# schmeing/ReSeq

Hardware: AMD Instinct MI355X
Metric: simulated read-pairs/sec (2x150 bp) (higher is better)
Workload: dtype f64

## Files before the change

reseq_amd/csrc/rsq_core.h:

```cpp
#pragma once
#include "rsq_types.h"
#if !defined(__HIPCC_RTC__)
#include <math.h>
#endif

namespace rsq {

struct Words {
    uint32_t w0, w1, w2, w3;
};


RSQ_HD Words philox(uint64_t seed, uint32_t c0, uint32_t c1, uint32_t c2, uint32_t c3) {
    uint32_t k0 = (uint32_t)seed, k1 = (uint32_t)(seed >> 32);
#pragma unroll
    for (int r = 0; r < 10; ++r) {
        const uint64_t p0 = (uint64_t)0xD2511F53u * c0, p1 = (uint64_t)0xCD9E8D57u * c2;
        const uint32_t hi0 = (uint32_t)(p0 >> 32), lo0 = (uint32_t)p0, hi1 = (uint32_t)(p1 >> 32), lo1 = (uint32_t)p1;
        c0 = hi1 ^ c1 ^ k0;
        c1 = lo1;
        c2 = hi0 ^ c3 ^ k1;
        c3 = lo0;
        k0 += 0x9E3779B9u;
        k1 += 0xBB67AE85u;
// ... 359 lines not shown
RSQ_HD void surrounding_forward(const uint64_t *__restrict__ words, uint64_t word_off, uint32_t L, uint32_t pos, uint32_t (&sur)[3],
                                const uint64_t *__restrict__ wrap_words = nullptr) {
    uint64_t p = (uint64_t)pos + L - kSurStart;
    if (p >= L) p -= L;
    bool wrapped = pos < kSurStart;
    if (p + kSurBlocks * kSurRange <= L) {
        const uint64_t x = ref_bits60(words, word_off, (uint32_t)p);
#pragma unroll
        for (uint32_t b = 0; b < kSurBlocks; ++b) sur[b] = reverse_ten_bases((uint32_t)(x >> (20u * b)) & 0xFFFFFu);
        return;
    }
#pragma unroll 1
    for (uint32_t b = 0; b < kSurBlocks; ++b) {
        uint32_t v = 0;
#pragma unroll 1
        for (uint32_t i = 0; i < kSurRange; ++i) {
            v = (v << 2) + ref_base(wrapped && wrap_words ? wrap_words : words, word_off, (uint32_t)p);
            if (++p == L) {
                p = 0;
                wrapped = !wrapped;
            }
        }
        sur[b] = v;
    }
}
RSQ_HD void surrounding_reverse(const uint64_t *__restrict__ words, uint64_t word_off, uint32_t L, uint32_t pos, uint32_t (&sur)[3],
                                const uint64_t *__restrict__ wrap_words = nullptr) {
    uint64_t q = (uint64_t)(L - pos - 1) + L - kSurStart;
    if (q >= L) q -= L;
    uint32_t f = L - 1u - (uint32_t)q;
    bool wrapped = pos + kSurStart >= L;
    if (f + 1u >= kSurBlocks * kSurRange) {
        const uint64_t x = ref_bits60(words, word_off, f + 1u - kSurBlocks * kSurRange);
#pragma unroll
        for (uint32_t b = 0; b < kSurBlocks; ++b) sur[b] = ~(uint32_t)(x >> (20u * (kSurBlocks - 1u - b))) & 0xFFFFFu;
        return;
    }
#pragma unroll 1
    for (uint32_t b = 0; b < kSurBlocks; ++b) {
        uint32_t v = 0;
#pragma unroll 1
        for (uint32_t i = 0; i < kSurRange; ++i) {
            v = (v << 2) + (3u - ref_base(wrapped && wrap_words ? wrap_words : words, word_off, f));
            if (f) --f;
            else {
                f = L - 1u;
                wrapped = !wrapped;
            }
        }
        sur[b] = v;
    }
}
RSQ_HD double surrounding_bias(const double *__restrict__ sur_bias, const uint32_t (&sur)[3]) {
    double bias = 0.0;
    for (int b = (int)kSurBlocks; b--;) bias += sur_bias[(size_t)b * kSurSize + sur[b]];
    return 2 / (1 + exp(-bias));
}

RSQ_HD double get_dispersion(double bias, double a, double b) {
    double r = bias / (a + b * bias);
    if (r > bias * 1e10) r = bias * 1e10;
    return r;
}
RSQ_HD uint32_t binomial(uint32_t n, double p, double probability_chosen) {
    double probability_count = pow(1 - p, (double)n), probability_left = probability_chosen - probability_count;
    uint32_t count = 0;
    while (0.0 < probability_left && count < n) {
        ++count;
        probability_count *= (double)(n + 1 - count) / count * p / (1 - p);
        probability_left -= probability_count;
    }
    return count;
}
RSQ_HD uint32_t negative_binomial(double p, double r, double probability_chosen) {
    double probability_count = pow(1 - p, r), probability_left = probability_chosen - probability_count;
    uint32_t count = 0;
    while (0.0 < probability_left) {
        count = (count + 1u) & 0xFFFFu;
        probability_count *= p * ((r - 1) / count + 1);
        probability_left -= probability_count;
    }
    return count;
}
RSQ_HD uint32_t fragment_counts(const DevSim &S, uint32_t seq, uint32_t fragment_length, uint32_t gc, const uint32_t (&sur_start)[3],
                                const uint32_t (&sur_end)[3], double probability_chosen) {
    double general = S.ref_seq_bias[seq] * S.insert_lengths_bias[fragment_length];
    double bias = general * S.gc_bias[gc] * surrounding_bias(S.sur_bias, sur_start) * surrounding_bias(S.sur_bias, sur_end);
    if (0.0 < bias) {
        double mean = bias * S.bias_normalization;
        double dispersion = get_dispersion(mean, S.dispersion[0], S.dispersion[1]) / S.num_alleles;
        mean /= S.num_alleles;
        return negative_binomial(mean / (mean + dispersion), dispersion, probability_chosen);
    }
    return 0;
}


RSQ_HD uint32_t digits10(uint32_t v) { return v < 10 ? 1u : v < 100 ? 2u : v < 1000 ? 3u : v < 10000 ? 4u : 5u; }

struct CigarRun {
    char element;
    uint32_t length;
    uint32_t chars;
    RSQ_HD void flush() { chars += digits10(length) + 1u; }
};

struct FillState {
    uint32_t read_length, read_pos;
    uint32_t previous_indel_type, indel_pos, base_call, gc_seq;
    uint32_t seq_qual, qual, error_rate, num_errors;
    uint32_t last_written_qual;
    uint32_t iteration;
};

RSQ_HD uint32_t draw_read_length(const DevSim &S, uint32_t seg, uint32_t fragment_length, double u) {
    const DevReadLengths &rl = S.read_lengths[seg];
    if (rl.fixed) return rl.fixed;
    const double random_value = u * (double)S.insert_lengths[fragment_length];
    double counter = 0.0;
    const uint32_t row = fragment_length - rl.row_first;
    const uint32_t from = rl.row_from[row] & 0xFFFFu;
    uint32_t read_len = (from + (rl.row_ptr[row + 1] - rl.row_ptr[row])) & 0xFFFFu;
    while (counter <= random_value) {
        const bool more = read_len > from;
        read_len = (read_len - 1u) & 0xFFFFu;
        if (!more) break;
        counter += (double)rl.values[rl.row_ptr[row] + (read_len - from)];
    }
    return read_len;
}

template <class Src>
RSQ_HD void template_totals_loop(const Src &src, uint32_t n, uint32_t &gc, uint32_t &rate_sum) {
    for (uint32_t k = 0; k < n; ++k) {
        if (is_gc(src.base(k))) ++gc;
        rate_sum += src.sys_base(k) >> 8;
    }
}

struct AdapterSrc {
    const uint8_t *seq;
    const uint16_t *sys_;
    RSQ_HD uint32_t base(uint32_t k) const { return seq[k]; }
    RSQ_HD uint32_t sys_base(uint32_t k) const { return sys_[k]; }
    RSQ_HD uint32_t sys_deleted(uint32_t k) const { return sys_[k]; }
};

struct ReadMachine {
    enum : uint32_t { kTemplate = 0, kAdapter = 1, kTail = 2, kDone = 3 };
    FillState par;
    CigarRun cg;
    uint32_t phase, seg, tile_id, tbase;
    uint32_t org_pos, org_len;
    uint32_t adapter_id, adapter_a0;
    uint32_t iter_m, hard_clip, tail_length, pos_tail, n_indels;
    uint32_t start_cut_word;

    RSQ_HD void idle() {
        par = FillState{};
        cg = CigarRun{'M', 0, 0};
        phase = kDone;
        seg = tile_id = tbase = org_pos = org_len = adapter_id = adapter_a0 = iter_m = hard_clip = tail_length = pos_tail = n_indels = start_cut_word = 0;
    }
    template <class Tab, class Src>
    RSQ_HD void init(const DevSim &S, const Tab &tab, const Stream &st, uint32_t seg_, uint32_t tile, uint32_t fragment_length, const Src &src) {
        seg = seg_;
        tile_id = tile;
        tbase = (seg * RSQ_SIM(S, n_tiles) + tile_id) * 4u;
        par.read_pos = 0;
        par.previous_indel_type = 0;
        par.indel_pos = 0;
        par.base_call = 5;
        par.gc_seq = 0;
        par.qual = 1;
        par.error_rate = 0;
        par.num_errors = 0;
        par.last_written_qual = 0;
// ... 198 lines not shown
```

reseq_amd/csrc/rsq_format.h:

```cpp
#pragma once
#include <string.h>

#include "rsq_reads.h"

namespace rsq {

RSQ_HD void image_or(RSQ_LDS uint32_t *w, uint32_t v) {
#if defined(__HIP_DEVICE_COMPILE__)
    __hip_atomic_fetch_or(w, v, __ATOMIC_RELAXED, __HIP_MEMORY_SCOPE_WORKGROUP);
#else
    uint32_t x;
    memcpy(&x, w, 4);
    x |= v;
    memcpy(w, &x, 4);
#endif
}
RSQ_HD uint32_t image_bytes_at(uint32_t hi, uint32_t lo, uint32_t at) {
#if defined(__HIP_DEVICE_COMPILE__)
    return __builtin_amdgcn_perm(hi, lo, 0x03020100u + at * 0x01010101u);
#else
    return (uint32_t)((((uint64_t)hi << 32) | lo) >> (8u * at));
#endif
}
RSQ_HD uint32_t image_word(const uint32_t *p) {
// ... 343 lines not shown
    const uint64_t i = (uint64_t)blockIdx.x * blockDim.x + threadIdx.x;
    if (i >= n) return;
    const uint32_t seg = segs[i] ? 1u : 0u, fl = frag_len[i];
    if (fl < range.lo[seg] || fl >= range.hi[seg]) atomicMin(first_bad, (uint32_t)i);
}
__global__ void k_record_flags(const uint8_t *segs, uint64_t n, uint32_t *flags) {
    const uint64_t i = (uint64_t)blockIdx.x * blockDim.x + threadIdx.x;
    if (i < n) flags[i] = segs[i] ? 1u : 0u;
}
__global__ void k_record_partition(const uint8_t *segs, uint64_t n, const uint64_t *ones_before, uint32_t *rec_index, uint32_t *rec_count) {
    const uint64_t i = (uint64_t)blockIdx.x * blockDim.x + threadIdx.x;
    const uint32_t n1 = (uint32_t)ones_before[n], n0 = (uint32_t)n - n1;
    if (i == 0) {
        rec_count[0] = n0;
        rec_count[1] = n1;
    }
    if (i >= n) return;
    const uint32_t before = (uint32_t)ones_before[i];
    if (segs[i]) rec_index[n0 + before] = (uint32_t)i;
    else rec_index[(uint32_t)i - before] = (uint32_t)i;
}

__global__ void __launch_bounds__(256) k_methylation_templates(DevSim S, const Fragment *frags, uint64_t n_pairs, RawLayout raw) {
    const uint64_t r = (uint64_t)blockIdx.x * blockDim.x + threadIdx.x;
    if (r >= 2u * n_pairs) return;
    const uint32_t seg = r >= n_pairs ? 1u : 0u;
    convert_template(S, frags[r - seg * n_pairs], seg, raw.templates + r * raw.template_words, raw.template_words);
}

__global__ void __launch_bounds__(256) k_variant_templates(DevSim S, const Fragment *frags, const FragmentVar *fvars, uint64_t n_pairs, RawLayout raw) {
    const uint64_t r = (uint64_t)blockIdx.x * blockDim.x + threadIdx.x;
    if (r >= 2u * n_pairs) return;
    const uint32_t seg = r >= n_pairs ? 1u : 0u;
    const uint64_t pair = r - seg * n_pairs;
    variant_template(S, frags[pair], fvars[pair], seg, raw.templates + r * raw.template_words, raw.template_words);
}

template <bool PERM, uint32_t ITEMS>
struct WaveImage {
    const uint64_t *offsets;
    char *dst;
    uint32_t lane, skew, bytes, slot_at;
    uint64_t row, item, g_begin;
    bool active, through_lds;
    static __device__ __forceinline__ uint64_t first() { return (uint64_t)blockIdx.x * ITEMS; }
    __device__ __forceinline__ WaveImage(const uint64_t *offsets, uint64_t n, char *dst, uint32_t lds_bytes, const uint32_t *perm, uint32_t lane) : offsets(offsets), dst(dst), lane(lane) {
        const uint64_t last = first() + ITEMS < n ? first() + ITEMS : n;
        row = first() + (lane & (ITEMS - 1u));
        active = row < last;
        item = PERM ? (active ? perm[row] : 0u) : row;
        g_begin = PERM ? (active ? offsets[item] : 0u) : offsets[first()];
        const uint64_t g_end = PERM ? (active ? offsets[item + 1u] : 0u) : offsets[last];
        skew = (uint32_t)((uint64_t)(uintptr_t)(dst + g_begin) & 15u);
        bytes = (uint32_t)(g_end - g_begin);
        const uint32_t slot = (lds_bytes / ITEMS) & ~15u;
        through_lds = PERM ? __all(skew + bytes <= slot) != 0 : skew + bytes <= lds_bytes;
        slot_at = PERM ? (lane & (ITEMS - 1u)) * slot : 0u;
    }
    __device__ __forceinline__ RSQ_LDS char *item_text(char *image) const { return (RSQ_LDS char *)image + slot_at + skew + (PERM ? 0u : (uint32_t)(offsets[item] - g_begin)); }
    __device__ __forceinline__ void clear(char *image, uint32_t lds_bytes) const {
        for (uint32_t c = lane * 16u; c < lds_bytes; c += 64u * 16u) *reinterpret_cast<uint4 *>(image + c) = uint4{0u, 0u, 0u, 0u};
        __syncthreads();
    }
    __device__ __forceinline__ void store_out(const char *image) const {
        __syncthreads();
        const uint32_t lo = skew, hi = skew + bytes;
        char *g_chunk0 = dst + g_begin - skew;
        const char *s_from = image + slot_at;
        for (uint32_t c = (PERM ? lane / ITEMS : lane) * 16u; c < hi; c += (PERM ? 64u / ITEMS : 64u) * 16u) {
            if (c >= lo && c + 16u <= hi) {
                *reinterpret_cast<uint4 *>(g_chunk0 + c) = *reinterpret_cast<const uint4 *>(s_from + c);
            } else {
                for (uint32_t b = c < lo ? lo : c; b < c + 16u && b < hi; ++b) g_chunk0[b] = s_from[b];
            }
        }
    }
};

constexpr uint32_t kFormatLdsMax = 16u * 1024u, kFormatLdsMin = 1024u;
RSQ_HD uint32_t format_lds_bytes(uint64_t record_bytes, bool slots) {
    const uint64_t want = (kFormatRecords * record_bytes + 16u + 127u) & ~(uint64_t)127u;
    const uint32_t image = (uint32_t)(want < kFormatLdsMin ? kFormatLdsMin : want > kFormatLdsMax ? kFormatLdsMax : want);
    return !slots ? image : image + 16u * kFormatRecords < kFormatLdsMax ? image + 16u * kFormatRecords : kFormatLdsMax;
}
__global__ void __launch_bounds__(256) k_max_size(const uint32_t *sizes, uint64_t n, uint32_t *longest) {
    uint32_t m = 0;
    for (uint64_t i = (uint64_t)blockIdx.x * blockDim.x + threadIdx.x; i < n; i += (uint64_t)gridDim.x * blockDim.x) m = max(m, sizes[i]);
    for (uint32_t d = 32; d; d >>= 1) m = max(m, (uint32_t)__shfl_xor((int)m, (int)d, 64));
    if ((threadIdx.x & 63u) == 0 && m) atomicMax(longest, m);
}
template <bool PERM>
__global__ void __launch_bounds__(64) k_format_write(DevSim S, NameTable names, const Fragment *frags, uint64_t n_pairs, uint64_t adapter_only_first, RawLayout raw,
                                                    const uint64_t *offsets0, const uint64_t *offsets1, char *dst0, char *dst1, uint64_t cap0, uint64_t cap1,
                                                    const FragmentVar *fvars, const uint32_t *perm, uint32_t lds_bytes) {
    extern __shared__ __attribute__((aligned(16))) char s_text[];
    using Image = WaveImage<PERM, kFormatRecords>;
    const uint32_t lane = threadIdx.x, seg = blockIdx.y, part = lane / kFormatRecords;
    if (Image::first() >= n_pairs) return;
    const uint64_t *offsets = seg ? offsets1 : offsets0;
    char *dst = seg ? dst1 : dst0;
    if (offsets[n_pairs] > (seg ? cap1 : cap0)) return;
    const Image im(offsets, n_pairs, dst, lds_bytes, perm, lane);
    const uint64_t pair = im.item;
    ReadMeta m;
    Fragment f;
    FragmentVar fv;
    uint64_t r = 0;
    if (im.active) {
        r = (uint64_t)seg * n_pairs + im.row;
        m = raw.meta[r];
        if (frags) f = frags[pair];
        if (frags && fvars) fv = fvars[pair];
    }
    const WordColumn seq = raw.seq_of(r), qual = raw.qual_of(r), ops = raw.ops_of(r);
    const uint64_t ao_number = adapter_only_first + pair + 1u;
    if (!im.through_lds) {
        if (im.active && part == 0u) format_record(S, names, frags != nullptr, f, ao_number, m, seq, qual, ops, dst + offsets[pair], frags && fvars, fv);
        return;
    }
    im.clear(s_text, lds_bytes);
    if (im.active) {
        const uint32_t header = (uint32_t)(offsets[pair + 1u] - offsets[pair]) - 2u * m.read_len - 4u;
        image_record_part(m, seq, qual, header, part, im.item_text(s_text), [&](ImageSink &t) { image_header(S, names, frags != nullptr, f, ao_number, m, ops, t, frags && fvars, fv); });
    }
    im.store_out(s_text);
}

RSQ_HD uint32_t error_model_record_size(const ReadMeta &m, uint32_t id_len) { return 1u + id_len + 1u + m.cigar_chars + 2u + digits_u32(m.num_errors) + 1u + 2u * m.read_len + 4u; }
struct RecordIds {
    const char *chars;
    const uint64_t *off;
    const uint32_t *at, *len;
    RSQ_HD const char *begin(uint64_t i) const { return chars + (off ? off[i] : (uint64_t)at[i] + 1u); }
    RSQ_HD uint32_t length(uint64_t i) const { return off ? (uint32_t)(off[i + 1] - off[i]) : len[i]; }
};
__global__ void __launch_bounds__(256) k_record_text_sizes(RawLayout raw, uint64_t n, RecordIds ids, uint32_t *sizes) {
    const uint64_t row = (uint64_t)blockIdx.x * blockDim.x + threadIdx.x;
    if (row >= n) return;
    const uint64_t i = raw.item_of(row);
    sizes[i] = error_model_record_size(raw.meta[row], ids.length(i));
}
template <bool PERM>
__global__ void __launch_bounds__(64) k_record_text_waves(RawLayout raw, uint64_t n, RecordIds ids, const uint64_t *offsets, char *dst, uint64_t cap, uint32_t lds_bytes) {
    extern __shared__ __attribute__((aligned(16))) char s_text[];
    using Image = WaveImage<PERM, kFormatRecords>;
    const uint32_t lane = threadIdx.x, part = lane / kFormatRecords;
    if (Image::first() >= n || offsets[n] > cap) return;
    const Image im(offsets, n, dst, lds_bytes, raw.order, lane);
    const uint64_t row = im.row, item = im.item;
    const bool active = im.active;
    ReadMeta m{};
    if (active) m = raw.meta[row];
    const WordColumn seq = raw.seq_of(active ? row : 0u), qual = raw.qual_of(active ? row : 0u), ops = raw.ops_of(active ? row : 0u);
    auto header = [&](auto &t) {
        t.ch('@');
        t.str(ids.begin(item), ids.length(item));
        t.ch(' ');
        cigar_replay(ops, m, t);
        t.str(" E", 2);
        t.num((uint32_t)m.num_errors);
        t.ch('\n');
    };
    auto image_head = [&](ImageSink &t) {
        t.str(ids.begin(item), ids.length(item), '@', ' ');
        cigar_replay(ops, m, t);
        t.push(chars4(' ', 'E'), 2u);
        t.num((uint32_t)m.num_errors, '\n', 1u);
    };
    if (!im.through_lds) {
        if (active && part == 0u) {
            WordSinkT<char *> t(dst + offsets[item]);
            header(t);
// ... 18 lines not shown
```

reseq_amd/csrc/rsq_host.cpp:

```cpp
#include <stdio.h>
#include "rsq_host.h"
#include "rsq_textio.h"

#include <errno.h>
#include <fcntl.h>
#include <string.h>
#include <sys/mman.h>
#include <sys/stat.h>
#include <unistd.h>
#include <zlib.h>

#include <algorithm>
#include <array>
#include <atomic>
#include <chrono>
#include <exception>
#include <memory>
#include <mutex>

#include <fstream>
#include <thread>

#include "rsq_core.h"

namespace rsq {

Options &options() {
    static Options o;
    return o;
}
namespace {
struct OptionEntry {
    const char *name;
    int64_t Options::*field;
};
const OptionEntry kOptionTable[] = {
    {"fill_mode", &Options::fill_mode},         {"image_tiles", &Options::image_tiles},     {"rate_rows", &Options::rate_rows},
    {"no_indel_skip", &Options::no_indel_skip}, {"force_exact", &Options::force_exact},     {"min_quality_quads", &Options::min_quality_quads},
    {"trace_plan", &Options::trace_plan},       {"trace_prepare", &Options::trace_prepare},
    {"bias_window", &Options::bias_window},     {"window_chunks", &Options::window_chunks}, {"serial_fasta", &Options::serial_fasta},   {"trace_load", &Options::trace_load},
    {"chain_chunk", &Options::chain_chunk},     {"chain_warmup", &Options::chain_warmup},
    {"serial_parse", &Options::serial_parse},   {"parse_stretch", &Options::parse_stretch}, {"mapped_parses", &Options::mapped_parses},
    {"fasta_stretch", &Options::fasta_stretch}, {"overlap", &Options::overlap}, {"specialize", &Options::specialize}, {"job_write_direct", &Options::job_write_direct},             {"job_chunk_bytes", &Options::job_chunk_bytes}, {"host_gzip", &Options::host_gzip}, {"fill_waves", &Options::fill_waves}, {"fasta_no_stage", &Options::fasta_no_stage},
    {"hiprtc_by_name", &Options::hiprtc_by_name}, {"gzip_route", &Options::gzip_route},       {"gzip_stretch", &Options::gzip_stretch},
};
}
bool set_option(const char *name, int64_t value) {
    for (const OptionEntry &e : kOptionTable)
        if (0 == strcmp(name, e.name)) {
            options().*(e.field) = value;
            return true;
        }
    return false;
}
bool get_option(const char *name, int64_t *value) {
    for (const OptionEntry &e : kOptionTable)
        if (0 == strcmp(name, e.name)) {
            *value = options().*(e.field);
            return true;
        }
    return false;
}
const char *option_names() {
    static const std::string names = [] {
        std::string s;
        for (const OptionEntry &e : kOptionTable) s += (s.empty() ? "" : " ") + std::string(e.name);
        return s;
    }();
    return names.c_str();
}

static size_t pad8(size_t n) { return (8 - (n & 7)) & 7; }

Container::Container(const std::string &path) {
    std::ifstream f(path, std::ios::binary | std::ios::ate);
    if (!f) throw Error("cannot open profile '" + path + "'");
    std::streamsize sz = f.tellg();
    f.seekg(0);
    buf_.resize((size_t)sz);
    if (!f.read(reinterpret_cast<char *>(buf_.data()), sz)) throw Error("cannot read profile '" + path + "'");
    if (buf_.size() < 16 || memcmp(buf_.data(), "RSQPROF1", 8) != 0) throw Error("'" + path + "' is not an RSQP profile container");
    uint32_t version, n;
    memcpy(&version, &buf_[8], 4);
    memcpy(&n, &buf_[12], 4);
    if (version != 1) throw Error("unsupported RSQP version");
    static const size_t kSize[7] = {1, 2, 4, 8, 4, 8, 8};
    size_t pos = 16;
    for (uint32_t i = 0; i < n; ++i) {
        if (pos + 4 > buf_.size()) throw Error("truncated RSQP container");
        uint16_t ln;
        memcpy(&ln, &buf_[pos], 2);
        std::string name(reinterpret_cast<const char *>(&buf_[pos + 2]), ln);
        Array a;
        a.dtype = buf_[pos + 2 + ln];
        int ndim = buf_[pos + 3 + ln];
        if (a.dtype > 6 || ndim > 4) throw Error("corrupt RSQP container");
        size_t head = (size_t)ln + 4;
        pos += head + pad8(head);
        a.count = 1;
        for (int d = 0; d < ndim; ++d) {
            uint64_t dim;
            memcpy(&dim, &buf_[pos], 8);
            a.dims.push_back(dim);
            a.count *= dim;
            pos += 8;
        }
        size_t nbytes = a.count * kSize[a.dtype];
        if (pos + nbytes > buf_.size()) throw Error("truncated RSQP container");
        a.data = &buf_[pos];
        pos += nbytes + pad8(nbytes);
        arrays_[name] = a;
    }
}

const Array &Container::get(const std::string &name) const {
    auto it = arrays_.find(name);
    if (it == arrays_.end()) throw Error("profile misses array '" + name + "'");
    return it->second;
}

std::vector<double> discrete_cp(const uint64_t *w, size_t n) {
    std::vector<double> cp(n ? n : 1, 1.0);
    if (n < 2) return cp;
    double sum = 0.0;
    for (size_t i = 0; i < n; ++i) sum += (double)w[i];
    double acc = 0.0;
    for (size_t i = 0; i < n; ++i) {
// ... 1174 lines not shown
```

reseq_amd/csrc/rsq_host.h:

```cpp
#pragma once
#include <stdint.h>

#include <map>
#include <stdexcept>
#include <string>
#include <string.h>
#include <vector>

namespace rsq {

struct Error : std::runtime_error {
    using std::runtime_error::runtime_error;
};

struct Options {
    int64_t fill_mode = -1;
    int64_t image_tiles = 0;
    int64_t rate_rows = 0;
    int64_t no_indel_skip = 0;
    int64_t force_exact = 0;
    int64_t min_quality_quads = 0;
    int64_t trace_plan = 0;
    int64_t trace_prepare = 0;
    int64_t bias_window = 0;
    int64_t window_chunks = 0;
    int64_t trace_load = 0;
    int64_t serial_fasta = 0;
    int64_t fasta_stretch = 0;
    int64_t chain_chunk = 0;
    int64_t chain_warmup = -1;
    int64_t serial_parse = 0;
    int64_t mapped_parses = 0;
    int64_t parse_stretch = 0;
    int64_t job_chunk_bytes = 0;
    int64_t job_write_direct = 0;
    int64_t specialize = 1;
    int64_t fasta_no_stage = 0;
    int64_t fill_waves = 0;
    int64_t host_gzip = 0;
    int64_t gzip_route = -1;
    int64_t gzip_stretch = 0;
    int64_t hiprtc_by_name = 0;
    int64_t overlap = 0;
};
Options &options();
bool set_option(const char *name, int64_t value);
bool get_option(const char *name, int64_t *value);
const char *option_names();

struct Array {
    int dtype = 0;
    std::vector<uint64_t> dims;
    uint64_t count = 0;
    const uint8_t *data = nullptr;
};

class Container {
   public:
    explicit Container(const std::string &path);
    const Array &get(const std::string &name) const;
    bool has(const std::string &name) const { return arrays_.count(name) != 0; }
    template <class T>
    std::vector<T> vec(const std::string &name, int dtype) const {
        const Array &a = get(name);
        if (a.dtype != dtype) throw Error("profile array '" + name + "' has the wrong type");
        const T *p = reinterpret_cast<const T *>(a.data);
        return std::vector<T>(p, p + a.count);
    }
    template <class T>
    T scalar(const std::string &name, int dtype) const {
        return vec<T>(name, dtype).at(0);
    }

   private:
    std::vector<uint8_t> buf_;
    std::map<std::string, Array> arrays_;
};

template <class T>
struct Vect {
    uint64_t from = 0;
    std::vector<T> v;
    uint64_t to() const { return from + v.size(); }
    T operator[](uint64_t i) const { return (i < from || i >= to()) ? T(0) : v[i - from]; }
};

struct HostTable {
    uint32_t nm = 0;
    std::vector<uint32_t> par0;
    uint32_t from[4] = {0, 0, 0, 0}, to[4] = {0, 0, 0, 0};
    std::vector<double> dim2[4];
    void modify_par0(uint32_t par0_index, double multiplier);
    void set_par0(uint32_t par0_index);
};

struct HostAdapters {
    std::vector<uint8_t> seqs;
    std::vector<uint32_t> seq_ptr;
    std::vector<uint64_t> counts, significant;
    std::vector<uint32_t> cut_ptr, cut_from;
    std::vector<uint64_t> cut;
    uint32_t n() const { return (uint32_t)seq_ptr.size() - 1; }
};

struct HostRlByFl {
    uint64_t from = 0;
    std::vector<uint32_t> row_ptr, row_from;
    std::vector<uint64_t> values, non_mapped;
};

struct Profile {
    uint8_t phred_offset = 33;
    double corrected_coverage = 0;
    uint16_t max_len_deletion = 0;
    uint32_t reset_distance = 0;
    Vect<uint64_t> read_lengths[2];
    HostRlByFl rl_by_fl[2];
    uint64_t total_number_reads = 0;
    std::vector<uint16_t> tiles;
    std::vector<uint64_t> tile_abundance;
    HostAdapters adapters[2];
    Vect<uint64_t> polya;
    uint64_t overrun_bases[5] = {0, 0, 0, 0, 0};
    Vect<uint64_t> insert_lengths;
    Vect<double> insert_lengths_bias, gc_bias;
// ... 104 lines not shown
```

reseq_amd/csrc/rsq_scan.h:

```cpp
#pragma once
#include "rsq_types.h"

namespace rsq {

#if RSQ_DEVICE_BUILD
constexpr uint32_t kScanBlock = 256;
constexpr uint32_t kScanPer = 8;
constexpr uint32_t kScanTile = kScanBlock * kScanPer;

__global__ void k_scan_tile_sums(const uint32_t *in, uint64_t n, uint64_t *tile_sums) {
    __shared__ uint64_t s[kScanBlock];
    uint64_t base = (uint64_t)blockIdx.x * kScanTile + (uint64_t)threadIdx.x * kScanPer, acc = 0;
    for (uint32_t i = 0; i < kScanPer; ++i)
        if (base + i < n) acc += in[base + i];
    s[threadIdx.x] = acc;
    __syncthreads();
    for (uint32_t d = kScanBlock / 2; d > 0; d >>= 1) {
        if (threadIdx.x < d) s[threadIdx.x] += s[threadIdx.x + d];
        __syncthreads();
    }
    if (threadIdx.x == 0) tile_sums[blockIdx.x] = s[0];
}
constexpr uint32_t kScanTilesBlock = 1024;
__global__ void __launch_bounds__(kScanTilesBlock) k_scan_tiles(uint64_t *tile_sums, uint32_t n_tiles, uint64_t *total, const uint64_t *init) {
    __shared__ uint64_t s[kScanTilesBlock];
    const uint64_t first = init ? *init : 0u;
    const uint32_t per = (n_tiles + kScanTilesBlock - 1u) / kScanTilesBlock, lo = threadIdx.x * per, hi = lo + per < n_tiles ? lo + per : n_tiles;
    uint64_t acc = 0;
    for (uint32_t i = lo; i < hi; ++i) acc += tile_sums[i];
    s[threadIdx.x] = acc;
    __syncthreads();
    for (uint32_t d = 1; d < kScanTilesBlock; d <<= 1) {
        const uint64_t v = threadIdx.x >= d ? s[threadIdx.x - d] : 0;
        __syncthreads();
        s[threadIdx.x] += v;
        __syncthreads();
    }
    uint64_t run = first + s[threadIdx.x] - acc;
    for (uint32_t i = lo; i < hi; ++i) {
        const uint64_t v = tile_sums[i];
        tile_sums[i] = run;
        run += v;
    }
    if (threadIdx.x == kScanTilesBlock - 1u) *total = first + s[threadIdx.x];
}
__global__ void k_scan_apply(const uint32_t *in, uint64_t n, const uint64_t *tile_sums, const uint64_t *total, uint64_t *out) {
    __shared__ uint64_t s[kScanBlock];
    const uint64_t base = (uint64_t)blockIdx.x * kScanTile + (uint64_t)threadIdx.x * kScanPer;
    uint32_t v[kScanPer];
    uint64_t acc = 0;
    for (uint32_t i = 0; i < kScanPer; ++i) {
        v[i] = base + i < n ? in[base + i] : 0u;
        acc += v[i];
    }
    s[threadIdx.x] = acc;
    __syncthreads();
    for (uint32_t d = 1; d < kScanBlock; d <<= 1) {
        uint64_t t = threadIdx.x >= d ? s[threadIdx.x - d] : 0;
        __syncthreads();
        s[threadIdx.x] += t;
        __syncthreads();
    }
    uint64_t run = tile_sums[blockIdx.x] + s[threadIdx.x] - acc;
    for (uint32_t i = 0; i < kScanPer; ++i) {
        if (base + i < n) out[base + i] = run;
        run += v[i];
    }
    if (blockIdx.x == 0 && threadIdx.x == 0) out[n] = *total;
}
#endif

}
```

reseq_amd/csrc/rsq_sieve.h:

```cpp
#pragma once
#include "rsq_core.h"
#include "rsq_variants.h"

namespace rsq {

struct SieveSite {
    uint32_t seq, start, L;
    uint64_t word_off;
    const double *thr;
    uint32_t group;
    uint32_t sur_start[3];
    bool have_start;
    uint32_t sub;
    VarStart st;
};

RSQ_HD uint32_t site_c1(const SieveSite &site) { return site.seq | (site.sub << 22); }

template <class F>
RSQ_HD uint32_t sieve_gaps(const DevSim &S, const SieveSite &site, F &&on_pass) {
    const double *q = S.gap_q + (size_t)site.group * S.insert_to;
    const uint32_t *seg_end = S.gap_seg_end + (size_t)site.group * S.insert_to;
    const uint32_t c1 = site_c1(site);
    uint32_t cur = S.insert_from, k = 0, n = 0;
    while (cur < S.insert_to) {
        const Words w = philox(S.seed, site.start, c1, k++, kDomSieve << 28);
        const uint32_t e = seg_end[cur];
        const double base = (cur == S.insert_from || seg_end[cur - 1u] == cur) ? 1.0 : q[cur - 1u];
        const double target = u53_to_unit(w.w0, w.w1) * base;
        uint32_t lo = cur, hi = e;
        while (lo < hi) {
            const uint32_t mid = (lo + hi) >> 1;
            if (q[mid] <= target) hi = mid;
            else lo = mid + 1u;
        }
        if (lo < e) {
            const double thr1 = site.thr[2u * lo + 1u];
            on_pass(lo, thr1 + u53_to_unit(w.w2, w.w3) * (1 - thr1));
            ++n;
            cur = lo + 1u;
        } else cur = e;
    }
    return n;
}

RSQ_HD uint32_t sieve_cell(const DevSim &S, SieveSite &site, uint32_t len, double probability_chosen, uint32_t (&cnt)[2], uint32_t (&strand_of)[2]) {
    cnt[0] = cnt[1] = 0;
    strand_of[0] = strand_of[1] = 0;
    const double thr0 = site.thr[2u * len], thr1 = site.thr[2u * len + 1u];
    if (!(probability_chosen >= thr1)) return 0;
    const uint32_t non_zero_strands = binomial(2u, 1 - thr0, probability_chosen);
    const uint32_t end = site.start + len;
    if (!non_zero_strands || !(end < site.L)) return 0;
    const Words w2 = philox(S.seed, site.start, site.seq, len, (kDomSieve << 28) | 1u);
    uint32_t n_chosen;
    if (non_zero_strands <= 1u) {
        strand_of[0] = (uint32_t)(u32_to_unit(w2.w2) * 2.0) & 1u;
        n_chosen = 1;
    } else {
        strand_of[0] = 0;
        strand_of[1] = 1;
        n_chosen = 2;
    }
    if (!site.have_start) {
        surrounding_forward(S.ref_words, site.word_off, site.L, site.start, site.sur_start);
        site.have_start = true;
    }
    uint32_t sur_end[3];
    surrounding_reverse(S.ref_words, site.word_off, site.L, end - 1u, sur_end);
    const uint32_t gc = percent_u32(ref_gc_count_prefix(S.ref_words, S.gc_prefix, site.word_off, site.start, end), len);
    uint32_t n_here = 0;
    for (uint32_t j = 0; j < n_chosen; ++j) {
        const double u = j ? u53_to_unit(w2.w2, w2.w3) : u53_to_unit(w2.w0, w2.w1);
        const double adjusted_random = thr0 + u * (1 - thr0);
        cnt[j] = fragment_counts(S, site.seq, len, gc, site.sur_start, sur_end, adjusted_random);
        n_here += cnt[j];
    }
    return n_here;
}

constexpr uint32_t kMaxDevAlleles = 128;
template <uint32_t CAP>
struct VarCellT {
    uint32_t n;
    uint16_t cnt[2 * CAP];
    uint8_t id[2 * CAP];
};
using VarCell = VarCellT<kMaxDevAlleles>;
template <uint32_t CAP>
struct SlotMaskT {
    static constexpr uint32_t kWords = (2 * CAP + 31) / 32;
    uint32_t w[kWords];
    RSQ_HD void set_first(uint32_t n) {
        for (uint32_t i = 0; i < kWords; ++i) w[i] = n >= 32u * (i + 1u) ? 0xFFFFFFFFu : (n > 32u * i ? (1u << (n - 32u * i)) - 1u : 0u);
    }
    RSQ_HD bool test(uint32_t id) const { return (w[id >> 5] >> (id & 31u)) & 1u; }
    RSQ_HD void clear(uint32_t id) { w[id >> 5] &= ~(1u << (id & 31u)); }
};
template <class Mask>
RSQ_HD void select_allele(uint8_t *chosen, uint32_t &n_chosen, Mask &selectable, uint32_t possible_strands, double random_value) {
    uint32_t chosen_id = (uint32_t)(uint16_t)(random_value * (possible_strands - n_chosen));
    uint32_t replacement_correction = 0;
    for (uint32_t i = 0; i < n_chosen; ++i)
        if (chosen[i] <= chosen_id) ++replacement_correction;
    while (replacement_correction)
        if (selectable.test(++chosen_id)) --replacement_correction;
    chosen[n_chosen++] = (uint8_t)chosen_id;
    selectable.clear(chosen_id);
}
RSQ_HD uint32_t word_of(const Words &w, uint32_t k) { return k == 0u ? w.w0 : (k == 1u ? w.w1 : (k == 2u ? w.w2 : w.w3)); }
template <uint32_t CAP>
RSQ_HD uint32_t sieve_cell_var(const DevSim &S, const SieveSite &site, uint32_t len, double probability_chosen, VarCellT<CAP> &cell) {
    cell.n = 0;
    const double thr0 = site.thr[2u * len], thr1 = site.thr[2u * len + 1u];
    if (!(probability_chosen >= thr1)) return 0;
    const uint32_t possible_strands = 2u * S.num_alleles;
    const uint32_t non_zero_strands = binomial(possible_strands, 1 - thr0, probability_chosen);
    const uint32_t end = site.start + len;
    if (!non_zero_strands || !(end < site.L)) return 0;
    uint8_t chosen[2 * CAP];
    uint32_t n_chosen = 0, n_draws = 0;
    SlotMaskT<CAP> selectable;
    selectable.set_first(possible_strands);
    const bool direct = non_zero_strands <= possible_strands / 2u;
    const uint32_t to_draw = direct ? non_zero_strands : possible_strands - non_zero_strands;
    Words ws{0, 0, 0, 0};
    while (n_chosen < to_draw) {
        if (0u == (n_draws & 3u)) ws = philox(S.seed, site.start, site.seq, len, (kDomSieve << 28) | (2u + (n_draws >> 2)));
        select_allele(chosen, n_chosen, selectable, possible_strands, u32_to_unit(word_of(ws, n_draws & 3u)));
        ++n_draws;
    }
    if (!direct) {
        n_chosen = 0;
        for (uint32_t id = 0; id < possible_strands; ++id)
            if (selectable.test(id)) chosen[n_chosen++] = (uint8_t)id;
    }
    uint32_t n_here = 0;
    Words wc{0, 0, 0, 0};
#pragma unroll 1
    for (uint32_t j = 0; j < n_chosen; ++j) {
        const uint32_t allele = chosen[j] >> 1;
        const uint64_t *words = hap_words(S, allele);
        uint32_t sur_start[3], sur_end[3];
        surrounding_forward(words, site.word_off, site.L, site.start, sur_start, S.ref_words);
        surrounding_reverse(words, site.word_off, site.L, end - 1u, sur_end, S.ref_words);
        const uint32_t gc = percent_u32(ref_gc_count_prefix(words, hap_gc_prefix(S, allele), site.word_off, site.start, end), len);
        if (0u == (j & 1u)) wc = philox(S.seed, site.start, site.seq, len, (kDomSieve << 28) | (128u + (j >> 1)));
        const double u = (j & 1u) ? u53_to_unit(wc.w2, wc.w3) : u53_to_unit(wc.w0, wc.w1);
        const double adjusted_random = thr0 + u * (1 - thr0);
        const uint32_t c = fragment_counts(S, site.seq, len, gc, sur_start, sur_end, adjusted_random);
        if (c) {
            cell.id[cell.n] = chosen[j];
            cell.cnt[cell.n] = (uint16_t)c;
            ++cell.n;
            n_here += c;
        }
    }
    return n_here;
}

template <uint32_t CAP>
// ... 107 lines not shown
    if constexpr (VM != 2) {
        const uint32_t block_id = block_lo + slot / kBlockSize;
        init_site(S, block_id, slot % kBlockSize, site);
        if (first_slot_of_block) *first_slot_of_block = slot - slot % kBlockSize;
        return block_id;
    } else {
        const uint32_t base_lo = S.block_extra_ptr[block_lo];
        uint32_t lo = block_lo, hi = block_hi;
        while (hi - lo > 1u) {
            const uint32_t mid = (lo + hi) >> 1;
            if ((mid - block_lo) * kBlockSize + (S.block_extra_ptr[mid] - base_lo) <= slot) lo = mid;
            else hi = mid;
        }
        const uint32_t block_id = lo, first = (block_id - block_lo) * kBlockSize + (S.block_extra_ptr[block_id] - base_lo), local = slot - first;
        if (first_slot_of_block) *first_slot_of_block = first;
        const ExtraStart *e = S.extra + S.block_extra_ptr[block_id];
        const uint32_t m = S.block_extra_ptr[block_id + 1] - S.block_extra_ptr[block_id];
        const uint32_t seq = S.block_seq[block_id], bs = (block_id - S.first_block[seq]) * kBlockSize;
        uint32_t a = 0, b = m;
        while (a < b) {
            const uint32_t mid = (a + b) >> 1;
            if ((e[mid].pos - bs) + mid + 1u < local) a = mid + 1u;
            else b = mid;
        }
        const uint32_t c = a;
        if (c < m && (e[c].pos - bs) + c + 1u == local) {
            init_site(S, block_id, e[c].pos - bs, site);
            site.sub = e[c].sub;
            site.st = VarStart{e[c].first_variant_id, e[c].start_variant_pos};
        } else {
            init_site(S, block_id, local - c, site);
            if (NEED_START && site.start < site.L) site.st = VarStart{(int32_t)var_view(S, seq).lower_bound(site.start), 0u};
        }
        return block_id;
    }
}

#if RSQ_DEVICE_BUILD
constexpr uint32_t kSieveBlock = 256;

__global__ void __launch_bounds__(256) k_slot_table(DevSim S, uint32_t block_lo, SlotInfo *out) {
    const uint32_t block_id = block_lo + blockIdx.x, base_lo = S.block_extra_ptr[block_lo];
    const uint32_t first_slot = (block_id - block_lo) * kBlockSize + (S.block_extra_ptr[block_id] - base_lo);
    const ExtraStart *e = S.extra + S.block_extra_ptr[block_id];
    const uint32_t m = S.block_extra_ptr[block_id + 1] - S.block_extra_ptr[block_id];
    const uint32_t seq = S.block_seq[block_id], bs = (block_id - S.first_block[seq]) * kBlockSize, L = S.seq_len[seq];
    const VarView r = var_view(S, seq);
    __shared__ uint32_t s_v[2];
    if (threadIdx.x < 2) s_v[threadIdx.x] = r.lower_bound(bs + threadIdx.x * kBlockSize);
    __syncthreads();
    const uint32_t v0 = s_v[0], v1 = s_v[1];
    for (uint32_t local = threadIdx.x; local < kBlockSize + m; local += blockDim.x) {
        uint32_t a = 0, b = m;
        while (a < b) {
            const uint32_t mid = (a + b) >> 1;
            if ((e[mid].pos - bs) + mid + 1u < local) a = mid + 1u;
            else b = mid;
        }
        SlotInfo t;
        t.block_id = block_id;
        t.first_slot = first_slot;
        if (a < m && (e[a].pos - bs) + a + 1u == local) {
            t.offset_in_block = e[a].pos - bs;
            t.sub = e[a].sub;
            t.first_variant_id = e[a].first_variant_id;
            t.start_variant_pos = e[a].start_variant_pos;
        } else {
            t.offset_in_block = local - a;
            t.sub = 0;
            const uint32_t pos = bs + t.offset_in_block;
            uint32_t lo = v0, hi = v1;
            while (lo < hi) {
                const uint32_t mid = (lo + hi) >> 1;
                if (r.v[mid].pos < pos) lo = mid + 1u;
                else hi = mid;
            }
            t.first_variant_id = pos < L ? (int32_t)lo : 0;
            t.start_variant_pos = 0;
        }
        out[first_slot + local] = t;
    }
}

template <int VM, bool FILL>
__global__ void __launch_bounds__(kSieveBlock) k_sieve_gaps(DevSim S, uint32_t block_lo, uint32_t block_hi, uint32_t n_slots, uint32_t *counts, const uint64_t *cand_off,
                                                            SieveCand *cands, uint64_t cand_cap, const SlotInfo *slots) {
    const uint32_t slot = blockIdx.x * kSieveBlock + threadIdx.x;
    if (slot >= n_slots) return;
    SieveSite site;
    init_site_slot<VM, false>(S, block_lo, block_hi, slot, site, nullptr, slots);
    if (!(site.start < site.L)) {
        if constexpr (!FILL) counts[slot] = 0;
        return;
    }
    if constexpr (FILL) {
        uint64_t at = cand_off[slot];
        sieve_gaps(S, site, [&](uint32_t len, double probability_chosen) {
            if (at < cand_cap) cands[at] = SieveCand{slot, len, probability_chosen};
            ++at;
        });
    } else counts[slot] = sieve_gaps(S, site, [](uint32_t, double) {});
}

template <int VM, uint32_t CAP = kMaxDevAlleles>
__global__ void __launch_bounds__(kSieveBlock) k_sieve_finish(DevSim S, uint32_t block_lo, uint32_t block_hi, uint32_t n_slots, const uint64_t *cand_off, const SieveCand *cands,
                                                              uint64_t cand_cap, uint32_t *pairs_of, SieveHit *hits, uint32_t hit_cap, uint32_t *hit_count, const SlotInfo *slots,
                                                              uint32_t *cell_info) {
    __shared__ uint32_t s_records, s_base;
    if (threadIdx.x == 0) s_records = 0;
    __syncthreads();
    const uint64_t c = (uint64_t)blockIdx.x * kSieveBlock + threadIdx.x;
    const bool has_cell = c < cand_cap && c < cand_off[n_slots];
    uint32_t n_here = 0, n_records = 0;
    SieveCand cand{};
    VarCellT<VM != 0 ? CAP : 1u> cell;
    cell.n = 0;
    if (has_cell) {
        cand = cands[c];
        SieveSite site;
        init_site_slot<VM>(S, block_lo, block_hi, cand.slot, site, nullptr, slots);
        if constexpr (VM == 2) n_here = sieve_cell_general(S, site, cand.len, cand.probability_chosen, cell);
        else if constexpr (VM == 1) n_here = sieve_cell_var(S, site, cand.len, cand.probability_chosen, cell);
        else {
            uint32_t cnt[2], strand_of[2];
            n_here = sieve_cell(S, site, cand.len, cand.probability_chosen, cnt, strand_of);
            cell.n = n_here ? 2u : 0u;
            for (uint32_t e = 0; e < 2u; ++e) {
                cell.cnt[e] = (uint16_t)cnt[e];
                cell.id[e] = (uint8_t)strand_of[e];
            }
        }
        n_records = (cell.n + 1u) / 2u;
    }
    if constexpr (VM == 0) {
        if (c < cand_cap) {
            pairs_of[c] = n_here;
            cell_info[c] = (uint32_t)cell.cnt[0] | ((uint32_t)(cell.id[0] & 1u) << 16) | ((uint32_t)(cell.id[1] & 1u) << 17);
        }
        return;
    }
    const uint32_t rank = n_records ? atomicAdd(&s_records, n_records) : 0u;
    __syncthreads();
    if (threadIdx.x == 0 && s_records) s_base = atomicAdd(hit_count, s_records);
    __syncthreads();
    uint32_t intra = 0;
    for (uint32_t e = 0; e < cell.n; e += 2u) {
        const bool two = e + 1u < cell.n;
        const uint32_t at = s_base + rank + e / 2u;
        SieveHit h;
        h.slot = cand.slot;
        h.cand = (uint32_t)c;
        h.intra = intra;
        h.len = (uint16_t)cand.len;
        h.cnt0 = cell.cnt[e];
        h.cnt1 = two ? cell.cnt[e + 1u] : (uint16_t)0;
        h.strand0 = cell.id[e] & 1u;
        h.allele0 = cell.id[e] >> 1;
        h.strand1 = two ? cell.id[e + 1u] & 1u : 0;
        h.allele1 = two ? cell.id[e + 1u] >> 1 : 0;
        if (at < hit_cap) hits[at] = h;
        intra += (uint32_t)h.cnt0 + h.cnt1;
    }
    if (c < cand_cap) pairs_of[c] = n_here;
}

template <int VM>
__global__ void __launch_bounds__(256) k_sieve_emit(DevSim S, uint32_t block_lo, uint32_t block_hi, const SieveHit *hits, uint32_t n_hits, const uint64_t *cand_off,
                                                   const uint64_t *pair_off, Fragment *frags, FragmentVar *fvars, const SlotInfo *slots, const SieveCand *cands = nullptr,
                                                   const uint32_t *pairs_of = nullptr, const uint32_t *cell_info = nullptr) {
    const uint32_t i = blockIdx.x * blockDim.x + threadIdx.x;
    if (i >= n_hits) return;
    SieveHit h;
    if constexpr (VM == 0) {
        const uint32_t pairs = pairs_of[i];
        if (!pairs) return;
        const SieveCand cand = cands[i];
        const uint32_t info = cell_info[i];
        h.slot = cand.slot;
        h.cand = i;
        h.intra = 0;
        h.len = (uint16_t)cand.len;
        h.cnt0 = (uint16_t)(info & 0xFFFFu);
        h.cnt1 = (uint16_t)(pairs - (info & 0xFFFFu));
        h.strand0 = (uint8_t)((info >> 16) & 1u);
        h.strand1 = (uint8_t)((info >> 17) & 1u);
        h.allele0 = h.allele1 = 0;
    } else h = hits[i];
    SieveSite site;
    uint32_t first_slot;
    const uint32_t block_id = init_site_slot<VM>(S, block_lo, block_hi, h.slot, site, &first_slot, slots);
    const uint64_t base = pair_off[h.cand];
    const uint32_t number_base = (uint32_t)(base - pair_off[cand_off[first_slot]]);
    uint32_t k = h.intra;
    for (uint32_t e = 0; e < 2u; ++e) {
        const uint32_t cnt = e ? h.cnt1 : h.cnt0, strand = e ? h.strand1 : h.strand0, allele = e ? h.allele1 : h.allele0;
        if (!cnt) continue;
        FragmentVar fv{};
        if constexpr (VM == 2) {
            const AlleleCell ac = allele_cell(allele_view(S, site.seq, allele), site.st, site.start, h.len);
            fv.end = ac.end;
            fv.sub = site.sub;
            fv.start_var = site.st.first_variant_id;
            fv.start_var_pos = site.st.start_variant_pos;
            fv.end_var = ac.end_var.first_variant_id;
            fv.end_var_pos = ac.end_var.start_variant_pos;
        }
        for (uint32_t dup = 0; dup < cnt; ++dup, ++k) {
            frags[base + k] = make_fragment(site, h.len, dup, strand, block_id, number_base + k + 1u, allele);
// ... 8 lines not shown
```

reseq_amd/csrc/rsq_sim.hip:

```cpp
#include <hip/hip_runtime.h>
#include <fcntl.h>
#include <sys/mman.h>
#include <sys/stat.h>
#include <math.h>
#include <string.h>
#include <unistd.h>

#include <algorithm>
#include <atomic>
#include <chrono>
#include <map>
#include <thread>
#include <memory>
#include <string>
#include <utility>
#include <vector>

#include "../../include/reseq_amd.h"
#include "rsq_deflate.h"
#include "rsq_fasta.h"
#include "rsq_chains.h"
#include "rsq_sieve.h"
#include "rsq_scan.h"
#include "rsq_text.h"
#include "rsq_reads.h"
#include "rsq_format.h"
#include "rsq_sam.h"
#include "rsq_bam.h"
#include "rsq_bamsort.h"
#include "rsq_pack.h"
#include "rsq_prepass.h"
#include "rsq_spec.h"
#include "rsq_textio.h"

namespace rsq {

static thread_local std::string g_last_error, g_last_warning;

struct HipError : Error {
    using Error::Error;
};
#define HIP_CHECK(expr)                                                                                       \
    do {                                                                                                      \
        hipError_t e_ = (expr);                                                                               \
        if (e_ != hipSuccess) throw HipError(std::string(#expr) + ": " + hipGetErrorString(e_));              \
    } while (0)

class DevBuf {
   public:
    DevBuf() = default;
    DevBuf(const DevBuf &) = delete;
    DevBuf &operator=(const DevBuf &) = delete;
    DevBuf(DevBuf &&o) noexcept : p_(o.p_), bytes_(o.bytes_) { o.p_ = nullptr; o.bytes_ = 0; }
    ~DevBuf() { if (p_) (void)hipFree(p_); }
    void reserve(size_t bytes) {
        if (bytes <= bytes_) return;
        if (p_) {
            HIP_CHECK(hipDeviceSynchronize());
            HIP_CHECK(hipFree(p_));
        }
        p_ = nullptr;
        bytes_ = 0;
        HIP_CHECK(hipMalloc(&p_, bytes ? bytes : 8));
        bytes_ = bytes;
    }
    template <class T>
    void upload(const std::vector<T> &v) {
        reserve(v.size() * sizeof(T) + 8);
        if (!v.empty()) HIP_CHECK(hipMemcpy(p_, v.data(), v.size() * sizeof(T), hipMemcpyHostToDevice));
    }
    void release() {
        if (p_) {
            HIP_CHECK(hipDeviceSynchronize());
            HIP_CHECK(hipFree(p_));
        }
        p_ = nullptr;
        bytes_ = 0;
    }
    void reserve_keeping(size_t bytes, size_t keep, hipStream_t st) {
        if (bytes <= bytes_) return;
        DevBuf bigger;
        bigger.reserve(bytes);
        if (keep) HIP_CHECK(hipMemcpyAsync(bigger.p_, p_, keep, hipMemcpyDeviceToDevice, st));
        HIP_CHECK(hipStreamSynchronize(st));
        std::swap(p_, bigger.p_);
        std::swap(bytes_, bigger.bytes_);
    }
    template <class T>
    T *as() const { return reinterpret_cast<T *>(p_); }
    size_t bytes() const { return bytes_; }

   private:
    void *p_ = nullptr;
    size_t bytes_ = 0;
};

}
#include "rsq_s2i.h"
namespace rsq {

struct Timer {
    std::vector<std::pair<hipEvent_t, hipEvent_t>> events;
    size_t used = 0;
    Timer() = default;
    Timer(const Timer &) = delete;
    Timer &operator=(const Timer &) = delete;
    ~Timer() {
        for (auto &e : events) {
            (void)hipEventDestroy(e.first);
            (void)hipEventDestroy(e.second);
        }
    }
    void reset() { used = 0; }
    void start(hipStream_t st) {
        if (used == events.size()) {
            hipEvent_t a, b;
            HIP_CHECK(hipEventCreate(&a));
            HIP_CHECK(hipEventCreate(&b));
            events.emplace_back(a, b);
        }
        HIP_CHECK(hipEventRecord(events[used].first, st));
    }
    void stop(hipStream_t st) {
        HIP_CHECK(hipEventRecord(events[used].second, st));
        ++used;
    }
    double ms() const {
        double sum = 0.0;
        for (size_t i = 0; i < used; ++i) {
            float t = 0;
            if (hipEventElapsedTime(&t, events[i].first, events[i].second) == hipSuccess) sum += t;
        }
        return sum;
    }
    size_t launches() const { return used; }
};

}

using namespace rsq;

struct rsq_profile {
    Profile p;
};
struct rsq_ref {
    Reference r;
    Variants variants;
    bool has_variants = false;
};

struct DeviceUploader : Uploader {
    std::vector<std::unique_ptr<DevBuf>> owned[kUploadScopes];
    int device = 0;
    void bind_thread() override { HIP_CHECK(hipSetDevice(device)); }
    void release_scope(int scope) override {
        HIP_CHECK(hipDeviceSynchronize());
        owned[scope].clear();
    }
    void *put_bytes(const void *data, size_t bytes) override {
        std::vector<std::unique_ptr<DevBuf>> &own = owned[current_scope];
        own.emplace_back(new DevBuf());
        own.back()->reserve(bytes + 8);
        HIP_CHECK(hipMemcpy(own.back()->as<void>(), data, bytes, hipMemcpyHostToDevice));
        return own.back()->as<void>();
    }
    void *put_zeros(size_t bytes) override {
        std::vector<std::unique_ptr<DevBuf>> &own = owned[current_scope];
        own.emplace_back(new DevBuf());
        own.back()->reserve(bytes + 8);
        HIP_CHECK(hipMemset(own.back()->as<void>(), 0, bytes + 8));
        return own.back()->as<void>();
    }
    void write_bytes(void *dst, const void *src, size_t bytes) override { HIP_CHECK(hipMemcpy(dst, src, bytes, hipMemcpyHostToDevice)); }
    void read_bytes(void *dst_host, const void *src, size_t bytes) override { HIP_CHECK(hipMemcpy(dst_host, src, bytes, hipMemcpyDeviceToHost)); }
};

struct MappedFile {
    const char *data = nullptr;
    size_t size = 0;
    explicit MappedFile(const char *path) {
        const int fd = open(path, O_RDONLY);
        if (fd < 0) throw Error(std::string("cannot open ") + path + ": " + strerror(errno));
        struct stat st;
        if (fstat(fd, &st) != 0 || st.st_size <= 0) {
            close(fd);
            throw Error(std::string(path) + " is empty or cannot be examined");
        }
        size = (size_t)st.st_size;
        void *p = mmap(nullptr, size, PROT_READ, MAP_PRIVATE, fd, 0);
        close(fd);
        if (p == MAP_FAILED) throw Error(std::string("cannot map ") + path);
        data = static_cast<const char *>(p);
    }
    ~MappedFile() {
        if (data) munmap(const_cast<char *>(data), size);
    }
    MappedFile(const MappedFile &) = delete;
    MappedFile &operator=(const MappedFile &) = delete;
};

struct rsq_sim : PrepassSim {
    int device = 0;
    DeviceUploader up;
    struct Workspace {
        DevBuf fvars;
        DevBuf slot_table;
        DevBuf counts, offsets, tile_sums, scan_total, frags, raw_seq, raw_qual, raw_ops, raw_meta, sizes, off_r1, off_r2, fill_counters, hits, hit_count, cands, pairs_of, pair_off, templates, rec_flags, rec_index, rec_count;
        DevBuf bin_keys, bin_small, bin_perm, bin_frags, bin_fvars;
        DevBuf fa_counts, fa_first, fa_at, fa_len, fa_id_len, fa_frag_len, fa_seg, fa_codes, fa_summary;
        DevBuf sam_sizes, sam_side, off_sam;
        DevBuf bam_side;
        DevBuf cell_info;
        hipEvent_t text_done = nullptr;
    } ws[2];
    struct JobText {
        std::vector<std::unique_ptr<DevBuf>> chunks[2];
        std::vector<size_t> used[2];
        uint64_t bytes[2] = {0, 0};
        bool complete = false;
        std::vector<unsigned char> packed[2];
        bool is_packed = false;
        bool device_packed = false;
        void clear() {
            complete = false;
            is_packed = false;
            device_packed = false;
            for (auto &p : packed) std::vector<unsigned char>().swap(p);
            for (int f = 0; f < 2; ++f) {
                chunks[f].clear();
                used[f].clear();
                bytes[f] = 0;
            }
        }
    } job;
    DevBuf totals;
    bool gz_dense = false;
    bool gz_keep_code = false, gz_have_code = false;
    DevBuf gz_slots, gz_sizes, gz_at, gz_hist, gz_codes, gz_total;
    Workspace *cur = &ws[0];
    hipStream_t side[2] = {nullptr, nullptr};
    hipEvent_t ev_call = nullptr, ev_fill = nullptr, ev_emit = nullptr;
    std::map<std::string, Timer> timers;
    uint32_t n_cu = 256;
    uint64_t *mailbox = nullptr;
    uint64_t format_record_bytes = 480;
    DevBuf longest_record;
    DevBuf sam_totals, sam_longest;
    uint64_t sam_pair_bytes = 1100;
    uint64_t bam_pair_bytes = 700;
    struct BamSorted {
        bool active = false;
        uint64_t stream_at = 0;
        uint32_t next_block = 0;
        uint64_t prev_cut = 0;
        BamSortPlan plan{};
        DevBuf stage[2], dir[2];
        int cur = 0;
        uint64_t n_held = 0, held_bytes = 0;
        uint64_t call_pairs = 0;
        uint32_t call_parts = 1;
        DevBuf keys[2], idx[2], hist, hist_at, sizes, at, flags, run_of, runs, result, out_of_order, windows, window_first;
        BamIndexState index;
    } bam_sorted;
    uint64_t record_text_bytes = 480;
    int force_fill_mode = -1;
    SpecKernels spec;
    std::string arch;
    bool specialize = true;
    struct ChainBufs {
        DevBuf chains, chunk_chain, used, out[2], changed, list;
    } chain_bufs;
};

static bool fill_is_binned(const rsq_sim &s) { return effective_fill_mask(s.dev.lds.mask, s.force_fill_mode) != 0 && s.dev.lds.binned; }
static thread_local std::string g_spec_note;
static hipFunction_t spec_kernel(rsq_sim &s, SpecKind kind, uint32_t mask, bool var, bool binned) {
    if (!s.specialize || mask == 0) return nullptr;
    std::string note;
    hipFunction_t fn = s.spec.get(s.dev, SpecVariant{kind, mask, var, binned}, s.arch, note);
    if (s.opt.trace_plan && note != g_spec_note) fprintf(stderr, "[rsq] %s\n", note.c_str());
    g_spec_note = note;
    return fn;
}

namespace rsq {

constexpr uint64_t kBiasWindow = 512ull << 20;
struct DevicePrepass : PrepassBackend {
    rsq_sim &s;
    hipStream_t st;
    DevicePrepass(rsq_sim &sim, void *stream) : s(sim), st((hipStream_t)stream) {}

    void bias_partials(const BiasPlan &plan, uint64_t g_lo, uint64_t g_hi, std::vector<double> &h_sum, std::vector<double> &h_max) override {
        const bool trace = s.opt.trace_prepare != 0;
        auto t0 = std::chrono::steady_clock::now();
        auto lap = [&](const char *what) {
            if (!trace) return;
            HIP_CHECK(hipStreamSynchronize(st));
            const auto t1 = std::chrono::steady_clock::now();
            fprintf(stderr, "prepare:   bias sums: %-18s %8.3f s\n", what, std::chrono::duration<double>(t1 - t0).count());
            t0 = t1;
        };
        const uint32_t n_chunks = bias_chunks(plan);
        if (!n_chunks) return;
        DevBuf d_params, d_chunk_param, d_chunk_ptr, d_sum, d_max, d_start_bias, d_end_bias;
        d_params.upload(plan.params);
        d_chunk_param.upload(plan.chunk_param);
        d_chunk_ptr.upload(plan.chunk_ptr);
        d_sum.reserve((size_t)n_chunks * 8);
        d_max.reserve((size_t)n_chunks * 8);
        HIP_CHECK(hipMemsetAsync(d_sum.as<double>(), 0, (size_t)n_chunks * 8, st));
        HIP_CHECK(hipMemsetAsync(d_max.as<double>(), 0, (size_t)n_chunks * 8, st));
        lap("chunk tables");
        const uint64_t lo = std::min<uint64_t>(g_lo, s.total_ref_size), hi = std::min<uint64_t>(g_hi, s.total_ref_size);
        uint64_t window = kBiasWindow;
        if (s.opt.bias_window > 0) window = (uint64_t)s.opt.bias_window;
        const uint64_t reach = (uint64_t)kBiasBlock * kBiasRun + s.dev.insert_to, track_len = std::min(hi - lo, window) + reach;
        d_start_bias.reserve(track_len * 8 + 16);
        d_end_bias.reserve(track_len * 8 + 16);
        lap("track buffers");
        for (uint64_t a = lo; a < hi; a += window) {
            const uint64_t b = std::min(hi, a + window), w_hi = std::min<uint64_t>(s.total_ref_size, b + reach);
            hipLaunchKernelGGL(k_surrounding_bias_tracks, dim3((uint32_t)cdiv(w_hi - a, 256)), dim3(256), 0, st, s.dev, d_start_bias.as<double>(), d_end_bias.as<double>(), a, w_hi);
            HIP_CHECK(hipGetLastError());
            hipLaunchKernelGGL(k_sum_bias, dim3(n_chunks), dim3(kBiasBlock), 0, st, s.dev, d_params.as<BiasParam>(), d_chunk_param.as<uint32_t>(), d_chunk_ptr.as<uint32_t>(),
                               d_start_bias.as<double>(), d_end_bias.as<double>(), a, d_sum.as<double>(), d_max.as<double>(), a, b);
            HIP_CHECK(hipGetLastError());
        }
        lap("track and sum kernels");
        HIP_CHECK(hipMemcpyAsync(h_sum.data(), d_sum.as<double>(), h_sum.size() * 8, hipMemcpyDeviceToHost, st));
        HIP_CHECK(hipMemcpyAsync(h_max.data(), d_max.as<double>(), h_max.size() * 8, hipMemcpyDeviceToHost, st));
        HIP_CHECK(hipStreamSynchronize(st));
        lap("download");
    }

    void begin_run(const ChainRun &run, const std::vector<uint32_t> &chunk_chain) override {
        rsq_sim::ChainBufs &b = s.chain_bufs;
        publish_chains(run);
        b.chunk_chain.upload(chunk_chain);
        b.used.reserve(run.n_chunks * 4);
        b.out[0].reserve(run.n_chunks * 4);
        b.out[1].reserve(run.n_chunks * 4);
        b.changed.reserve(8);
        b.list.reserve((size_t)run.n_chunks * 4 + 16);
    }
    void publish_chains(const ChainRun &run) override { s.chain_bufs.chains.upload(run.chains); }
    uint32_t run_pass(const ChainRun &run, uint32_t pass, int prev, int cur) override {
        rsq_sim::ChainBufs &b = s.chain_bufs;
        uint32_t *out_prev = b.out[prev].as<uint32_t>(), *out_new = b.out[cur].as<uint32_t>();
        uint32_t n_run = run.n_chunks;
        const uint32_t *list = nullptr;
        if (pass > 0) {
            HIP_CHECK(hipMemsetAsync(b.changed.as<uint32_t>(), 0, 4, st));
            hipLaunchKernelGGL(k_sys_chain_select, dim3(cdiv(run.n_chunks, 256)), dim3(256), 0, st, b.chains.as<Chain>(), b.chunk_chain.as<uint32_t>(), run.n_chunks,
                               b.used.as<uint32_t>(), out_prev, out_new, b.list.as<uint32_t>(), b.changed.as<uint32_t>(), (int)pass);
            HIP_CHECK(hipGetLastError());
            HIP_CHECK(hipMemcpyAsync(&n_run, b.changed.as<uint32_t>(), 4, hipMemcpyDeviceToHost, st));
            HIP_CHECK(hipStreamSynchronize(st));
            list = b.list.as<uint32_t>();
        }
        if (n_run) {
            hipLaunchKernelGGL(k_sys_chain, dim3(cdiv(n_run, 64)), dim3(64), 0, st, s.dev, b.chains.as<Chain>(), b.chunk_chain.as<uint32_t>(), list, n_run, s.chain_chunk,
                               chain_warmup_len(s.chain_chunk, s.opt), b.used.as<uint32_t>(), out_prev, out_new, (int)pass);
            HIP_CHECK(hipGetLastError());
        }
        return n_run;
    }
    uint32_t out_state(const ChainRun &, int cur, size_t chunk) override {
        uint32_t state = 0;
        HIP_CHECK(hipMemcpy(&state, s.chain_bufs.out[cur].as<uint32_t>() + chunk, 4, hipMemcpyDeviceToHost));
        return state;
    }
    void variant_sys_errors(const ChainRun &run) override {
        const uint32_t n_variants = (uint32_t)s.variants.size();
        if (!s.has_variants || !n_variants) return;
        std::vector<ChainSpan> span((size_t)s.dev.n_seqs * 2, ChainSpan{-1, 0});
        for (size_t c = 0; c < run.chains.size(); ++c) {
            const Chain &ch = run.chains[c];
            if (ch.kind > 1u) continue;
            span[(size_t)ch.id * 2 + ch.kind] = ChainSpan{(int32_t)c, (c + 1 < run.chains.size() ? run.chains[c + 1].first_chunk : run.n_chunks) - ch.first_chunk};
        }
        DevBuf d_span, d_states;
        d_span.upload(span);
        d_states.reserve((size_t)n_variants * 8);
        hipLaunchKernelGGL(k_variant_chain_states, dim3(cdiv(n_variants, 256), 2), dim3(256), 0, st, s.dev, s.chain_bufs.chains.as<Chain>(), d_span.as<ChainSpan>(),
                           s.chain_bufs.used.as<uint32_t>(), s.chain_chunk, n_variants, d_states.as<uint32_t>());
        HIP_CHECK(hipGetLastError());
        std::vector<uint32_t> states((size_t)n_variants * 2);
        HIP_CHECK(hipMemcpyAsync(states.data(), d_states.as<uint32_t>(), states.size() * 4, hipMemcpyDeviceToHost, st));
        HIP_CHECK(hipStreamSynchronize(st));
        const std::vector<StrandTask> windows = strand_tasks(s.opt, run.chains, run.n_chunks, s.chain_chunk, [](uint32_t) { return 0u; });
        build_variant_sys_errors(s, s.up, &windows, states.data(), states.data() + n_variants);
    }
    void ready_to_simulate() override {
        if (s.has_ref) (void)spec_kernel(s, SpecKind::kReads, effective_fill_mask(s.dev.lds.mask, s.force_fill_mode), s.has_variants, fill_is_binned(s));
    }
};

static void exclusive_scan(rsq_sim &s, const uint32_t *in, uint64_t n, uint64_t *out, hipStream_t st, const uint64_t *init = nullptr, uint64_t *total_out = nullptr) {
    const uint32_t tiles = cdiv(n, kScanTile);
    s.cur->tile_sums.reserve((size_t)(tiles + 1) * 8);
    s.cur->scan_total.reserve(8);
    uint64_t *total = total_out ? total_out : s.cur->scan_total.as<uint64_t>();
    hipLaunchKernelGGL(k_scan_tile_sums, dim3(tiles), dim3(kScanBlock), 0, st, in, n, s.cur->tile_sums.as<uint64_t>());
    hipLaunchKernelGGL(k_scan_tiles, dim3(1), dim3(kScanTilesBlock), 0, st, s.cur->tile_sums.as<uint64_t>(), tiles, total, init);
    hipLaunchKernelGGL(k_scan_apply, dim3(tiles), dim3(kScanBlock), 0, st, in, n, s.cur->tile_sums.as<uint64_t>(), total, out);
    HIP_CHECK(hipGetLastError());
}

static RawLayout raw_layout(rsq_sim &s, uint64_t n_reads) {
    const uint64_t pitch = (n_reads + 63u) & ~(uint64_t)63u;
    s.cur->raw_seq.reserve((uint64_t)(s.read_stride / 4u) * pitch * 4 + 16);
    s.cur->raw_qual.reserve((uint64_t)(s.read_stride / 4u) * pitch * 4 + 16);
    s.cur->raw_ops.reserve((uint64_t)s.ops_stride * pitch * 4 + 16);
    s.cur->raw_meta.reserve(n_reads * sizeof(ReadMeta) + 16);
    return RawLayout{s.cur->raw_seq.as<uint32_t>(), s.cur->raw_qual.as<uint32_t>(), s.cur->raw_ops.as<uint32_t>(), s.cur->raw_meta.as<ReadMeta>(), pitch, nullptr, 0, nullptr};
}

template <class CountKernel>
static FillBins build_fill_bins(rsq_sim &s, uint64_t n_items, uint32_t n_keys, hipStream_t st, CountKernel &&count_keys, const Fragment *frags = nullptr,
                                const FragmentVar *fvars = nullptr) {
    if (n_items >= 0xFFFFFFFFull) throw Error("more than 2^32 reads in one call of a profile with tiles: use smaller block ranges");
    const uint32_t n_bins = 2 * s.dev.n_tiles;
    s.cur->bin_keys.reserve(n_items * 2 + 16);
    s.cur->bin_perm.reserve(n_items * 4 + 16);
    const size_t words = 2 * (size_t)n_keys + 5 * (size_t)n_bins + 1;
    s.cur->bin_small.reserve(words * 4 + 16);
    uint32_t *hist = s.cur->bin_small.as<uint32_t>(), *cursor = hist + n_keys, *bin_first = cursor + n_keys, *bin_count = bin_first + n_bins, *next_chunk = bin_count + n_bins,
             *workers = next_chunk + n_bins, *chunk_ptr = workers + n_bins;
    HIP_CHECK(hipMemsetAsync(hist, 0, (size_t)n_keys * 4, st));
    s.timers["bin_tiles"].start(st);
    count_keys(s.cur->bin_keys.as<uint16_t>(), hist);
    hipLaunchKernelGGL(k_bins_plan, dim3(1), dim3(1024), 0, st, hist, n_keys, n_bins, bin_first, bin_count, cursor, chunk_ptr, next_chunk, workers);
    if (frags) s.cur->bin_frags.reserve(n_items * sizeof(Fragment) + 16);
    if (fvars) s.cur->bin_fvars.reserve(n_items * sizeof(FragmentVar) + 16);
    hipLaunchKernelGGL(k_bin_scatter, dim3(cdiv(n_items, kBinBlock * kBinItemsPerThread)), dim3(kBinBlock), 0, st, s.cur->bin_keys.as<uint16_t>(), n_items, n_keys, cursor,
                       s.cur->bin_perm.as<uint32_t>(), frags, fvars, s.cur->bin_frags.as<Fragment>(), s.cur->bin_fvars.as<FragmentVar>());
    s.timers["bin_tiles"].stop(st);
    HIP_CHECK(hipGetLastError());
    return FillBins{s.cur->bin_perm.as<uint32_t>(), bin_first, bin_count, chunk_ptr, next_chunk, workers, n_bins, s.cur->bin_frags.as<Fragment>(), s.cur->bin_fvars.as<FragmentVar>()};
}
static void spec_allow_lds(hipFunction_t fn, size_t lds_bytes) {
    if (lds_bytes > 64 * 1024 && hipFuncSetAttribute(reinterpret_cast<const void *>(fn), hipFuncAttributeMaxDynamicSharedMemorySize, (int)lds_bytes) != hipSuccess) (void)hipGetLastError();
}
template <class Kernel>
static size_t fill_lds_bytes(const rsq_sim &s, bool screened, bool binned, Kernel kernel) {
    const size_t lds_bytes = (screened ? (size_t)s.dev.lds.total_words * 4u : 0) + (binned ? kSchedWords * 4u : 0);
    if (lds_bytes > 64 * 1024) HIP_CHECK(hipFuncSetAttribute(reinterpret_cast<const void *>(kernel), hipFuncAttributeMaxDynamicSharedMemorySize, (int)lds_bytes));
    return lds_bytes;
}
struct FillShape {
    uint32_t blocks, threads;
};
static FillShape fill_shape(const rsq_sim &s, size_t lds_bytes, uint64_t n_items, uint32_t segments_per_item, uint32_t max_threads) {
    const uint32_t per_cu = lds_bytes * 2 <= kLdsBudgetBytes ? 2u : 1u;
    const uint64_t chunks = segments_per_item * ((n_items + 63) / 64), slots = (uint64_t)s.n_cu * per_cu;
    uint32_t waves = (uint32_t)std::min<uint64_t>(max_threads / 64u, std::max<uint64_t>(4u, cdiv(chunks, slots)));
    waves = std::min(max_threads / 64u, (waves + 3u) & ~3u);
    if (s.opt.fill_waves > 0) waves = (uint32_t)std::min<int64_t>(max_threads / 64u, s.opt.fill_waves);
    const uint32_t blocks = (uint32_t)std::min<uint64_t>(slots, std::max<uint64_t>(2, cdiv(chunks, waves)));
    return FillShape{(blocks + 1u) & ~1u, waves * 64u};
}

template <class LaunchOwn>
static void launch_read_kernel(rsq_sim &s, hipStream_t st, const FillShape &shape, size_t lds_bytes, size_t counter_bytes, hipFunction_t spec, void **args, uint32_t *&counters,
                               LaunchOwn &&launch_own) {
    s.cur->fill_counters.reserve(counter_bytes);
    counters = s.cur->fill_counters.as<uint32_t>();
    HIP_CHECK(hipMemsetAsync(counters, 0, counter_bytes, st));
    s.timers["fill_reads"].start(st);
    if (spec) {
        spec_allow_lds(spec, lds_bytes);
        HIP_CHECK(hipModuleLaunchKernel(spec, shape.blocks, 1, 1, shape.threads, 1, 1, (unsigned)lds_bytes, st, args, nullptr));
    } else launch_own();
    s.timers["fill_reads"].stop(st);
    HIP_CHECK(hipGetLastError());
}
template <uint32_t MASK, bool VAR, bool BINNED>
static const uint32_t *launch_fill_kernel(rsq_sim &s, const Fragment *frags, uint64_t n_pairs, uint64_t adapter_first, const RawLayout &raw, hipStream_t st, const FragmentVar *fvars) {
    FillBins bins{};
    if (BINNED)
        bins = build_fill_bins(s, n_pairs, s.dev.n_tiles, st, [&](uint16_t *keys, uint32_t *hist) {
            hipLaunchKernelGGL(k_pair_tiles, dim3(cdiv(n_pairs, kBinBlock)), dim3(kBinBlock), 0, st, s.dev, frags, fvars, n_pairs, adapter_first, keys, hist);
        }, frags, fvars);
    const size_t lds_bytes = fill_lds_bytes(s, MASK != 0, BINNED, &k_fill_reads<MASK, VAR, BINNED>);
    const FillShape shape = fill_shape(s, lds_bytes, n_pairs, 2, fill_block(VAR));
    uint32_t *sizes = s.cur->sizes.as<uint32_t>(), *counters = nullptr;
    RawLayout raw_arg = raw;
    void *args[] = {&s.dev, &s.names, &frags, &n_pairs, &adapter_first, &raw_arg, &sizes, &counters, &fvars, &bins};
    launch_read_kernel(s, st, shape, lds_bytes, 8, spec_kernel(s, SpecKind::kReads, MASK, VAR, BINNED), args, counters, [&] {
// ... 44 lines not shown
            run += t[4 + 4 * b] - t[3 + 4 * b];
        }
        if (getenv("RSQ_TRACE_WORKGROUPS")) {
            std::string line;
            for (uint32_t b = 0; b < blocks; ++b) {
                line += " " + std::to_string(b) + ":" + std::to_string((t[2 + 4 * b] - first) / 100) + "+" + std::to_string((t[4 + 4 * b] - t[2 + 4 * b]) / 100) + "/" + std::to_string(t[5 + 4 * b]);
            }
            fprintf(stderr, "trace_fill workgroup:start+duration(us)/chunks:%s\n", line.c_str());
        }
        fprintf(stderr, "trace_fill: %u workgroups of %u threads, %llu items: last start %.1f us after the first, last end %.1f us; image staged in %.1f us, chunks %.1f us (means; 100 MHz clock)\n", blocks,
                shape.threads, (unsigned long long)n, (last_start - first) / 100.0, (last_end - first) / 100.0, stage / 100.0 / blocks, run / 100.0 / blocks);
    }
#endif
    return bins.perm;
}
template <uint32_t MASK>
static const uint32_t *launch_records_mask(rsq_sim &s, const RecordJob &job, const uint8_t *seg_dev, uint64_t n, const RawLayout &raw, hipStream_t st) {
    if constexpr (MASK != 0)
        if (fill_is_binned(s)) return job.codes ? launch_records_kernel<MASK, true, true>(s, job, seg_dev, n, raw, st) : launch_records_kernel<MASK, true, false>(s, job, seg_dev, n, raw, st);
    return job.codes ? launch_records_kernel<MASK, false, true>(s, job, seg_dev, n, raw, st) : launch_records_kernel<MASK, false, false>(s, job, seg_dev, n, raw, st);
}
template <class F, size_t... I>
static const uint32_t *with_fill_mask(uint32_t mask, const char *kernel, F &&f, std::index_sequence<I...>) {
    const uint32_t *order = nullptr;
    auto tried = [&](auto q) { return mask == q() && (order = f(q), true); };
    if (!(tried(std::integral_constant<uint32_t, 0u>{}) || ... || tried(std::integral_constant<uint32_t, kQualityQuads[I]>{})))
        throw Error(std::string("no ") + kernel + " instantiation for " + std::to_string(mask) + " quads");
    return order;
}
template <class F>
static const uint32_t *with_fill_mask(rsq_sim &s, const char *kernel, F &&f) {
    return with_fill_mask(effective_fill_mask(s.dev.lds.mask, s.force_fill_mode), kernel, f, std::make_index_sequence<sizeof(kQualityQuads) / sizeof(kQualityQuads[0])>{});
}
static const uint32_t *launch_fill_reads(rsq_sim &s, const Fragment *frags, uint64_t n_pairs, uint64_t adapter_first, const RawLayout &raw, hipStream_t st,
                              const FragmentVar *fvars = nullptr) {
    const bool var = frags && s.has_variants;
    return with_fill_mask(s, "k_fill_reads", [&](auto q) {
        if (var) return launch_fill_mask<decltype(q)::value, true>(s, frags, n_pairs, adapter_first, raw, st, fvars);
        return launch_fill_mask<decltype(q)::value>(s, frags, n_pairs, adapter_first, raw, st);
    });
}
static const uint32_t *launch_fill_records(rsq_sim &s, const RecordJob &job, const uint8_t *seg_dev, uint64_t n, const RawLayout &raw, hipStream_t st) {
    return with_fill_mask(s, "k_fill_records", [&](auto q) { return launch_records_mask<decltype(q)::value>(s, job, seg_dev, n, raw, st); });
}

template <class K, class... A>
static void launch_text_waves(K with_order, K in_order, const uint32_t *row_order, dim3 grid, uint32_t lds, hipStream_t st, A... args) {
    hipLaunchKernelGGL(row_order ? with_order : in_order, grid, dim3(64), lds, st, args...);
}

struct ReadsDone {
    RawLayout raw;
    const uint32_t *row_order;
};
static ReadsDone reads_stage(rsq_sim &s, const Fragment *frags, uint64_t n_pairs, uint64_t adapter_first, hipStream_t st, const FragmentVar *fvars) {
    RawLayout raw = raw_layout(s, 2 * n_pairs);
    s.cur->sizes.reserve(2 * n_pairs * 4 + 16);
    if (frags && s.dev.meth_ptr && !fvars) {
        s.cur->templates.reserve(2 * n_pairs * s.template_words * 8 + 16);
        raw.templates = s.cur->templates.as<uint64_t>();
        raw.template_words = s.template_words;
        hipLaunchKernelGGL(k_methylation_templates, dim3(cdiv(2 * n_pairs, 256)), dim3(256), 0, st, s.dev, frags, n_pairs, raw);
        HIP_CHECK(hipGetLastError());
    }
    if (frags && fvars) {
        s.cur->templates.reserve(2 * n_pairs * s.template_words * 8 + 16);
        raw.templates = s.cur->templates.as<uint64_t>();
        raw.template_words = s.template_words;
        s.timers["variant_templates"].start(st);
        hipLaunchKernelGGL(k_variant_templates, dim3(cdiv(2 * n_pairs, 256)), dim3(256), 0, st, s.dev, frags, fvars, n_pairs, raw);
        s.timers["variant_templates"].stop(st);
        HIP_CHECK(hipGetLastError());
    }
    const uint32_t *row_order = launch_fill_reads(s, frags, n_pairs, adapter_first, raw, st, fvars);
    return ReadsDone{raw, row_order};
}
static void text_stage(rsq_sim &s, const Fragment *frags, uint64_t n_pairs, uint64_t adapter_first, const ReadsDone &rd, char *r1, size_t r1_cap, char *r2, size_t r2_cap,
                       uint32_t part, hipStream_t st, const FragmentVar *fvars) {
    rsq_sim::Workspace &w = *s.cur;
    w.off_r1.reserve((n_pairs + 1) * 8);
    w.off_r2.reserve((n_pairs + 1) * 8);
    uint64_t *totals = s.totals.as<uint64_t>();
    s.timers["scan"].start(st);
    exclusive_scan(s, w.sizes.as<uint32_t>(), n_pairs, w.off_r1.as<uint64_t>(), st, totals + 2 * part, totals + 2 * (part + 1));
    exclusive_scan(s, w.sizes.as<uint32_t>() + n_pairs, n_pairs, w.off_r2.as<uint64_t>(), st, totals + 2 * part + 1, totals + 2 * (part + 1) + 1);
    s.timers["scan"].stop(st);
    const uint32_t lds = format_lds_bytes(s.format_record_bytes, rd.row_order != nullptr);
    hipLaunchKernelGGL(k_max_size, dim3(std::min<uint64_t>(1024, cdiv(2 * n_pairs, 256))), dim3(256), 0, st, w.sizes.as<uint32_t>(), 2 * n_pairs, s.longest_record.as<uint32_t>());
    s.timers["format_write"].start(st);
    launch_text_waves(k_format_write<true>, k_format_write<false>, rd.row_order, dim3(cdiv(n_pairs, kFormatRecords), 2), lds, st, s.dev, s.names, frags, n_pairs, adapter_first, rd.raw,
                      w.off_r1.as<uint64_t>(), w.off_r2.as<uint64_t>(), r1, r2, (uint64_t)(r1 ? r1_cap : 0), (uint64_t)(r2 ? r2_cap : 0), fvars, rd.row_order, lds);
    s.timers["format_write"].stop(st);
    HIP_CHECK(hipGetLastError());
}
struct SamOut {
    char *dst;
    size_t cap;
    size_t *len;
    bool bam = false;
    bool sorted = false;
};
static char *sorted_stage_room(rsq_sim &s, uint64_t n_pairs, uint32_t part, hipStream_t st, uint64_t &cap) {
    rsq_sim::BamSorted &b = s.bam_sorted;
    uint64_t ends[2];
    HIP_CHECK(hipMemcpyAsync(ends, s.sam_totals.as<uint64_t>() + part, 16, hipMemcpyDeviceToHost, st));
    HIP_CHECK(hipStreamSynchronize(st));
    const uint64_t bytes = b.held_bytes + ends[1] + 32u, entries = b.n_held + 2u * (b.call_pairs + n_pairs);
    const uint64_t left = b.call_parts > part + 1u ? b.call_parts - (part + 1u) : 0u;
    if (bytes > b.stage[b.cur].bytes()) {
        const uint64_t whole = bytes + (ends[1] - ends[0]) * left;
        b.stage[b.cur].reserve_keeping(whole + whole / 8u, b.held_bytes + ends[0], st);
    }
    if (entries * sizeof(BamDirEntry) > b.dir[b.cur].bytes()) {
        const uint64_t whole = entries + 2u * n_pairs * left;
        b.dir[b.cur].reserve_keeping((whole + whole / 8u) * sizeof(BamDirEntry), (b.n_held + 2u * b.call_pairs) * sizeof(BamDirEntry), st);
    }
    cap = b.stage[b.cur].bytes() - 32u - b.held_bytes;
    return b.stage[b.cur].as<char>() + b.held_bytes;
}
static void sorted_directory(rsq_sim &s, const Fragment *frags, uint64_t n_pairs, const ReadsDone &rd, const BamPair *side, const uint64_t *offsets, hipStream_t st) {
    rsq_sim::BamSorted &b = s.bam_sorted;
    s.timers["bam_sort_keys"].start(st);
    hipLaunchKernelGGL(k_bam_sort_keys, dim3(cdiv(n_pairs, 256)), dim3(256), 0, st, frags, n_pairs, rd.row_order, side, offsets, b.held_bytes,
                       b.dir[b.cur].as<BamDirEntry>() + b.n_held + 2u * b.call_pairs, s.dev.n_seqs, b.prev_cut, b.plan.pos_bits, b.out_of_order.as<uint32_t>());
    s.timers["bam_sort_keys"].stop(st);
    HIP_CHECK(hipGetLastError());
    b.call_pairs += n_pairs;
}
template <class Format>
static void truth_stage(rsq_sim &s, const Fragment *frags, uint64_t n_pairs, uint64_t adapter_first, const ReadsDone &rd, char *r1, size_t r1_cap, char *r2, size_t r2_cap, const SamOut &sam,
                        uint32_t part, hipStream_t st) {
    using Pair = typename Format::Pair;
    constexpr bool bam = std::is_same<Format, BamFormat>::value;
    const char *sizes_timer = bam ? "bam_sizes" : "sam_sizes", *write_timer = bam ? "bam_write" : "sam_write";
    rsq_sim::Workspace &w = *s.cur;
    DevBuf &side = bam ? w.bam_side : w.sam_side;
    w.sam_sizes.reserve(n_pairs * 4 + 16);
    w.off_sam.reserve((n_pairs + 1) * 8);
    side.reserve(n_pairs * sizeof(Pair) + 16);
    uint64_t *totals = s.sam_totals.as<uint64_t>();
    char *dst = sam.dst;
    uint64_t cap = sam.dst ? sam.cap : 0;
    const uint64_t cap1 = r1 ? r1_cap : 0, cap2 = r2 ? r2_cap : 0;
    s.timers[sizes_timer].start(st);
    hipLaunchKernelGGL(k_truth_sizes<Format>, dim3(cdiv(n_pairs, 256)), dim3(256), 0, st, s.dev, s.names, frags, n_pairs, adapter_first, rd.raw, rd.row_order, side.as<Pair>(),
                       w.sam_sizes.as<uint32_t>());
    s.timers[sizes_timer].stop(st);
    exclusive_scan(s, w.sam_sizes.as<uint32_t>(), n_pairs, w.off_sam.as<uint64_t>(), st, totals + part, totals + part + 1);
    hipLaunchKernelGGL(k_max_size, dim3(std::min<uint64_t>(1024, cdiv(n_pairs, 256))), dim3(256), 0, st, w.sam_sizes.as<uint32_t>(), n_pairs, s.sam_longest.as<uint32_t>());
    const uint32_t lds = sam_lds_bytes(bam ? s.bam_pair_bytes : s.sam_pair_bytes, rd.row_order != nullptr);
    if (sam.sorted) dst = sorted_stage_room(s, n_pairs, part, st, cap);
    s.timers[write_timer].start(st);
    launch_text_waves(k_truth_write<Format, true>, k_truth_write<Format, false>, rd.row_order, dim3(cdiv(n_pairs, kSamPairs)), lds, st, s.dev, s.names, frags, n_pairs, adapter_first, rd.raw,
                      side.as<Pair>(), w.off_sam.as<uint64_t>(), dst, cap, w.off_r1.as<uint64_t>() + n_pairs, w.off_r2.as<uint64_t>() + n_pairs, cap1, cap2, rd.row_order, lds);
    s.timers[write_timer].stop(st);
    HIP_CHECK(hipGetLastError());
    if constexpr (bam)
        if (sam.sorted) sorted_directory(s, frags, n_pairs, rd, side.as<Pair>(), w.off_sam.as<uint64_t>(), st);
}
static void sam_stage(rsq_sim &s, const Fragment *frags, uint64_t n_pairs, uint64_t adapter_first, const ReadsDone &rd, char *r1, size_t r1_cap, char *r2, size_t r2_cap, const SamOut &sam,
                      uint32_t part, hipStream_t st) {
    (sam.bam ? truth_stage<BamFormat> : truth_stage<SamFormat>)(s, frags, n_pairs, adapter_first, rd, r1, r1_cap, r2, r2_cap, sam, part, st);
}
static void begin_sam_totals(rsq_sim &s, uint32_t parts, hipStream_t st) {
    s.sam_totals.reserve((size_t)(parts + 1) * 8 + 16);
    s.sam_longest.reserve(8);
    HIP_CHECK(hipMemsetAsync(s.sam_totals.as<uint64_t>(), 0, 8, st));
    HIP_CHECK(hipMemsetAsync(s.sam_longest.as<uint32_t>(), 0, 4, st));
}
static void enqueue_sam_total(rsq_sim &s, uint32_t parts, hipStream_t text_stream) {
    HIP_CHECK(hipMemcpyAsync(&s.mailbox[6], s.sam_totals.as<uint64_t>() + parts, 8, hipMemcpyDeviceToHost, text_stream));
    s.mailbox[7] = 0;
    HIP_CHECK(hipMemcpyAsync(&s.mailbox[7], s.sam_longest.as<uint32_t>(), 4, hipMemcpyDeviceToHost, text_stream));
}
static int finish_sam(rsq_sim &s, int rc, const SamOut &sam, size_t r1_len, size_t r2_len) {
    *sam.len = s.mailbox[6];
    if ((uint32_t)s.mailbox[7]) (sam.bam ? s.bam_pair_bytes : s.sam_pair_bytes) = (uint32_t)s.mailbox[7] + 16u;
    if (sam.sorted) return rc;
    if (rc == RSQ_ENOSPC || (rc == RSQ_OK && (*sam.len > sam.cap || !sam.dst))) {
        g_last_error = "output buffers too small: need " + std::to_string(r1_len) + " and " + std::to_string(r2_len) + " bytes of FASTQ text and " + std::to_string(*sam.len) +
                       (sam.bam ? " of BAM records" : " of SAM text");
        return RSQ_ENOSPC;
    }
    return rc;
}
static void reset_call_timers(rsq_sim &s) {
    for (auto &t : s.timers) t.second.reset();
}
static int finish_call(rsq_sim &s, uint32_t parts, bool with_variants, char *r1, size_t r1_cap, size_t *r1_len, char *r2, size_t r2_cap, size_t *r2_len, hipStream_t text_stream) {
    s.mailbox[4] = 0;
    if (with_variants) HIP_CHECK(hipMemcpyAsync(&s.mailbox[4], s.dev.walk_error, 4, hipMemcpyDeviceToHost, text_stream));
    HIP_CHECK(hipMemcpyAsync(&s.mailbox[2], s.totals.as<uint64_t>() + 2 * parts, 16, hipMemcpyDeviceToHost, text_stream));
    HIP_CHECK(hipMemcpyAsync(&s.mailbox[5], s.longest_record.as<uint32_t>(), 4, hipMemcpyDeviceToHost, text_stream));
    HIP_CHECK(hipStreamSynchronize(text_stream));
    *r1_len = s.mailbox[2];
    *r2_len = s.mailbox[3];
    if ((uint32_t)s.mailbox[4]) {
        HIP_CHECK(hipMemsetAsync(s.dev.walk_error, 0, 4, text_stream));
        HIP_CHECK(hipStreamSynchronize(text_stream));
        g_last_error = kWalkErrorMessage;
        return RSQ_EINVAL;
    }
    if (*r1_len > r1_cap || *r2_len > r2_cap || !r1 || !r2) {
        g_last_error = "output buffers too small: need " + std::to_string(*r1_len) + " and " + std::to_string(*r2_len) + " bytes";
        return RSQ_ENOSPC;
    }
    return RSQ_OK;
}
static void begin_totals(rsq_sim &s, uint32_t parts, hipStream_t st) {
    s.totals.reserve((size_t)(parts + 1) * 16 + 16);
    s.longest_record.reserve(8);
    HIP_CHECK(hipMemsetAsync(s.totals.as<uint64_t>(), 0, 16, st));
    HIP_CHECK(hipMemsetAsync(s.longest_record.as<uint32_t>(), 0, 4, st));
}

static int adapter_only_pairs(rsq_sim &s, uint64_t n_pairs, uint64_t adapter_first, char *r1, size_t r1_cap, size_t *r1_len, char *r2, size_t r2_cap, size_t *r2_len, hipStream_t st,
                              const SamOut *sam = nullptr) {
    *r1_len = *r2_len = 0;
    if (sam) *sam->len = 0;
    if (!n_pairs) return RSQ_OK;
    reset_call_timers(s);
    s.cur = &s.ws[0];
    begin_totals(s, 1, st);
    if (sam) begin_sam_totals(s, 1, st);
    const ReadsDone rd = reads_stage(s, nullptr, n_pairs, adapter_first, st, nullptr);
    text_stage(s, nullptr, n_pairs, adapter_first, rd, r1, r1_cap, r2, r2_cap, 0, st, nullptr);
    if (sam) {
        sam_stage(s, nullptr, n_pairs, adapter_first, rd, r1, r1_cap, r2, r2_cap, *sam, 0, st);
        enqueue_sam_total(s, 1, st);
    }
    const int rc = finish_call(s, 1, false, r1, r1_cap, r1_len, r2, r2_cap, r2_len, st);
    return sam ? finish_sam(s, rc, *sam, *r1_len, *r2_len) : rc;
}

struct SieveRun {
    uint32_t block_lo = 0, block_hi = 0;
    uint64_t n_slots = 0, cand_cap = 0, hit_cap = 0, total = 0, n_cands = 0;
    uint32_t n_hits = 0;
    const SlotInfo *slot_table = nullptr;
};
static void sieve_attempt(rsq_sim &s, SieveRun &r, int attempt, uint64_t *mail, hipStream_t st) {
    rsq_sim::Workspace &w = *s.cur;
    const int vm = s.variants_mode;
    if (r.cand_cap >= (1ull << 32)) throw Error("more than 2^32 sieve candidates in one call: use smaller block ranges");
    w.cands.reserve(r.cand_cap * sizeof(SieveCand));
    w.pairs_of.reserve(r.cand_cap * 4 + 16);
    w.pair_off.reserve((r.cand_cap + 1) * 8);
    if (vm) w.hits.reserve(r.hit_cap * sizeof(SieveHit));
    else w.cell_info.reserve(r.cand_cap * 4 + 16);
    HIP_CHECK(hipMemsetAsync(w.hit_count.as<uint32_t>(), 0, 4, st));
    s.timers["sieve"].start(st);
    const uint32_t block_lo = r.block_lo, block_hi = r.block_hi;
    const uint64_t n_slots = r.n_slots, cand_cap = r.cand_cap;
    const dim3 ggrid(cdiv(n_slots, kSieveBlock)), gblock(kSieveBlock);
    if (!attempt) {
        if (2 == vm) {
            w.slot_table.reserve(n_slots * sizeof(SlotInfo) + 16);
            s.timers["slot_table"].start(st);
            hipLaunchKernelGGL(k_slot_table, dim3(block_hi - block_lo), dim3(256), 0, st, s.dev, block_lo, w.slot_table.as<SlotInfo>());
            s.timers["slot_table"].stop(st);
            r.slot_table = w.slot_table.as<SlotInfo>();
        }
        s.timers["sieve_screen"].start(st);
        if (2 == vm)
            hipLaunchKernelGGL((k_sieve_gaps<2, false>), ggrid, gblock, 0, st, s.dev, block_lo, block_hi, (uint32_t)n_slots, w.counts.as<uint32_t>(), (const uint64_t *)nullptr,
                               (SieveCand *)nullptr, cand_cap, r.slot_table);
        else
            hipLaunchKernelGGL((k_sieve_gaps<0, false>), ggrid, gblock, 0, st, s.dev, block_lo, block_hi, (uint32_t)n_slots, w.counts.as<uint32_t>(), (const uint64_t *)nullptr,
                               (SieveCand *)nullptr, cand_cap, r.slot_table);
        s.timers["sieve_screen"].stop(st);
        exclusive_scan(s, w.counts.as<uint32_t>(), n_slots, w.offsets.as<uint64_t>(), st);
    }
    const SlotInfo *slot_table = r.slot_table;
    if (2 == vm)
        hipLaunchKernelGGL((k_sieve_gaps<2, true>), ggrid, gblock, 0, st, s.dev, block_lo, block_hi, (uint32_t)n_slots, (uint32_t *)nullptr, w.offsets.as<uint64_t>(),
                           w.cands.as<SieveCand>(), cand_cap, slot_table);
    else
        hipLaunchKernelGGL((k_sieve_gaps<0, true>), ggrid, gblock, 0, st, s.dev, block_lo, block_hi, (uint32_t)n_slots, (uint32_t *)nullptr, w.offsets.as<uint64_t>(),
                           w.cands.as<SieveCand>(), cand_cap, slot_table);
    const dim3 fgrid(cdiv(cand_cap, kSieveBlock)), fblock(kSieveBlock);
#define RSQ_FINISH(VM, CAP)                                                                                                                                   \
    hipLaunchKernelGGL((k_sieve_finish<VM, CAP>), fgrid, fblock, 0, st, s.dev, block_lo, block_hi, (uint32_t)n_slots, w.offsets.as<uint64_t>(), w.cands.as<SieveCand>(),  \
                       cand_cap, w.pairs_of.as<uint32_t>(), w.hits.as<SieveHit>(), (uint32_t)std::min<uint64_t>(r.hit_cap, 0xFFFFFFFFull), w.hit_count.as<uint32_t>(), slot_table, \
                       w.cell_info.as<uint32_t>())
    if (2 == vm && s.num_alleles <= 8) RSQ_FINISH(2, 8);
    else if (2 == vm) RSQ_FINISH(2, kMaxDevAlleles);
    else if (1 == vm) RSQ_FINISH(1, 8);
    else RSQ_FINISH(0, 1);
#undef RSQ_FINISH
    s.timers["sieve"].stop(st);
    HIP_CHECK(hipGetLastError());
    exclusive_scan(s, w.pairs_of.as<uint32_t>(), cand_cap, w.pair_off.as<uint64_t>(), st);
    mail[1] = 0;
    HIP_CHECK(hipMemcpyAsync(&mail[0], w.pair_off.as<uint64_t>() + cand_cap, 8, hipMemcpyDeviceToHost, st));
    HIP_CHECK(hipMemcpyAsync(&mail[1], w.hit_count.as<uint32_t>(), 4, hipMemcpyDeviceToHost, st));
    HIP_CHECK(hipMemcpyAsync(&mail[5], w.offsets.as<uint64_t>() + n_slots, 8, hipMemcpyDeviceToHost, st));
}
static bool sieve_launch(rsq_sim &s, SieveRun &r, uint32_t block_lo, uint32_t block_hi, uint64_t *mail, hipStream_t st) {
    rsq_sim::Workspace &w = *s.cur;
    const int vm = s.variants_mode;
    r = SieveRun{};
    r.block_lo = block_lo;
    r.block_hi = block_hi;
    r.n_slots = (uint64_t)(block_hi - block_lo) * kBlockSize;
    if (2 == vm && block_hi > block_lo) {
        uint32_t ptr[2];
        HIP_CHECK(hipMemcpy(&ptr[0], s.dev.block_extra_ptr + block_lo, 4, hipMemcpyDeviceToHost));
        HIP_CHECK(hipMemcpy(&ptr[1], s.dev.block_extra_ptr + block_hi, 4, hipMemcpyDeviceToHost));
        r.n_slots += ptr[1] - ptr[0];
    }
    if (!r.n_slots) return false;
    if (r.n_slots >= (1ull << 32) - kSieveBlock)
        throw Error("block range too large for one call: at most " + std::to_string(((1ull << 32) - kSieveBlock) / kBlockSize - 1) + " blocks");
    w.counts.reserve(r.n_slots * 4 + 16);
    w.offsets.reserve((r.n_slots + 1) * 8);
    w.hit_count.reserve(8);
    const double expected_cands = s.expected_passing * (double)r.n_slots;
    r.cand_cap = std::max<uint64_t>(w.cands.bytes() / sizeof(SieveCand), (uint64_t)(expected_cands + 6.0 * sqrt(expected_cands + 1.0)) + 65536);
    r.hit_cap = std::max<uint64_t>(w.hits.bytes() / sizeof(SieveHit), 0 == vm ? r.cand_cap : r.cand_cap + r.cand_cap / 4);
    sieve_attempt(s, r, 0, mail, st);
    return true;
}
static void sieve_collect(rsq_sim &s, SieveRun &r, uint64_t *mail, hipStream_t st) {
    for (int attempt = 0;; ++attempt) {
        HIP_CHECK(hipStreamSynchronize(st));
        r.total = mail[0];
        r.n_hits = (uint32_t)mail[1];
        r.n_cands = mail[5];
        if (r.n_cands <= r.cand_cap && r.n_hits <= r.hit_cap) return;
        if (attempt >= 2) throw Error("sieve lists overflowed three times");
        const double grow = r.n_cands > r.cand_cap ? (double)r.n_cands / (double)r.cand_cap : 1.0;
        if (r.n_hits > r.hit_cap || grow > 1.0) r.hit_cap = std::max<uint64_t>(r.hit_cap, (uint64_t)((double)r.n_hits * grow * 1.25) + 65536);
        r.cand_cap = std::max(r.cand_cap, r.n_cands + 65536);
        sieve_attempt(s, r, attempt + 1, mail, st);
    }
}
static void sieve_emit(rsq_sim &s, const SieveRun &r, hipStream_t st) {
    rsq_sim::Workspace &w = *s.cur;
    w.frags.reserve(r.total * sizeof(Fragment) + 16);
    s.timers["sieve_emit"].start(st);
    if (2 == s.variants_mode) {
        w.fvars.reserve(r.total * sizeof(FragmentVar) + 16);
        hipLaunchKernelGGL(k_sieve_emit<2>, dim3(cdiv(r.n_hits, 256)), dim3(256), 0, st, s.dev, r.block_lo, r.block_hi, w.hits.as<SieveHit>(), r.n_hits, w.offsets.as<uint64_t>(),
                           w.pair_off.as<uint64_t>(), w.frags.as<Fragment>(), w.fvars.as<FragmentVar>(), w.slot_table.as<SlotInfo>());
    } else if (1 == s.variants_mode)
        hipLaunchKernelGGL(k_sieve_emit<1>, dim3(cdiv(r.n_hits, 256)), dim3(256), 0, st, s.dev, r.block_lo, r.block_hi, w.hits.as<SieveHit>(), r.n_hits, w.offsets.as<uint64_t>(),
                           w.pair_off.as<uint64_t>(), w.frags.as<Fragment>(), (FragmentVar *)nullptr, (const SlotInfo *)nullptr);
    else
        hipLaunchKernelGGL(k_sieve_emit<0>, dim3(cdiv(r.n_cands, 256)), dim3(256), 0, st, s.dev, r.block_lo, r.block_hi, (const SieveHit *)nullptr, (uint32_t)r.n_cands,
                           w.offsets.as<uint64_t>(), w.pair_off.as<uint64_t>(), w.frags.as<Fragment>(), (FragmentVar *)nullptr, (const SlotInfo *)nullptr, w.cands.as<SieveCand>(),
                           w.pairs_of.as<uint32_t>(), w.cell_info.as<uint32_t>());
    s.timers["sieve_emit"].stop(st);
    HIP_CHECK(hipGetLastError());
}

static uint32_t pairs_parts(const rsq_sim &s, uint32_t n_blocks) {
    const int64_t opt = s.opt.overlap;
    return opt > 0 ? (uint32_t)std::min<int64_t>(opt, std::max<uint32_t>(n_blocks, 1u)) : 1u;
}
static int check_block_range(const rsq_sim &s, uint32_t block_lo, uint32_t block_hi) {
    if (!s.prepared || !s.has_ref) {
        g_last_error = "rsq_sim_prepare with a reference must run before rsq_sim_pairs";
        return RSQ_ESTATE;
    }
    if (block_lo < 1 || block_hi > s.total_blocks + 1 || block_lo > block_hi) {
        g_last_error = "block range outside [1, total_blocks]";
        return RSQ_EINVAL;
// ... 551 lines not shown
int rsq_ref_write_fasta(const rsq_ref *r, const char *path) {
    REQUIRE(r && path, "null argument");
    try {
        std::string text;
        for (size_t i = 0; i < r->r.codes.size(); ++i) {
            text += '>';
            text += r->r.names[i];
            text += '\n';
            const std::vector<uint8_t> &c = r->r.codes[i];
            for (size_t k = 0; k < c.size(); k += 70) {
                for (size_t j = k; j < std::min(c.size(), k + 70); ++j) text += "ACGTN"[c[j] < 4 ? c[j] : 4];
                text += '\n';
            }
        }
        write_text_file(path, text);
        return RSQ_OK;
    } catch (const std::exception &e) {
        g_last_error = e.what();
        return RSQ_EIO;
    }
}
int rsq_ref_get_codes(const rsq_ref *r, uint32_t seq, uint8_t *out, uint32_t len) {
    REQUIRE(r && out && seq < r->r.codes.size() && len == r->r.codes[seq].size(), "bad sequence id or length");
    memcpy(out, r->r.codes[seq].data(), len);
    return RSQ_OK;
}

int rsq_sim_create(const rsq_profile *p, const rsq_ref *ref, int device, rsq_sim **out) {
    REQUIRE(p && out, "null argument");
    int n = rsq_device_count();
    if (n < 0) return n;
    REQUIRE(device >= 0 && device < n, "device index out of range");
    std::unique_ptr<rsq_sim> s(new rsq_sim());
    int rc = guard([&] {
        HIP_CHECK(hipSetDevice(device));
        s->device = device;
        s->up.device = device;
        hipDeviceProp_t prop;
        HIP_CHECK(hipGetDeviceProperties(&prop, device));
        s->n_cu = (uint32_t)prop.multiProcessorCount;
        s->arch = prop.gcnArchName;
        s->specialize = s->opt.specialize != 0;
        HIP_CHECK(hipHostMalloc(reinterpret_cast<void **>(&s->mailbox), 16 * sizeof(uint64_t), hipHostMallocDefault));
        for (hipStream_t &st : s->side) HIP_CHECK(hipStreamCreateWithFlags(&st, hipStreamNonBlocking));
        for (rsq_sim::Workspace &w : s->ws) HIP_CHECK(hipEventCreateWithFlags(&w.text_done, hipEventDisableTiming));
        HIP_CHECK(hipEventCreateWithFlags(&s->ev_call, hipEventDisableTiming));
        HIP_CHECK(hipEventCreateWithFlags(&s->ev_fill, hipEventDisableTiming));
        HIP_CHECK(hipEventCreateWithFlags(&s->ev_emit, hipEventDisableTiming));
        s->force_fill_mode = (int)s->opt.fill_mode;
        s->prof = p->p;
        pack_tables(*s, s->up);
        g_last_warning = s->plan_note;
        pack_profile(*s, s->up);
        if (ref) pack_reference(*s, s->up, ref->r, ref->has_variants ? &ref->variants : nullptr);
        return RSQ_OK;
    });
    if (rc == RSQ_OK) *out = s.release();
    return rc;
}
int rsq_sim_take_options(rsq_sim *s) {
    REQUIRE(s, "null argument");
    s->opt = options();
    return RSQ_OK;
}
void rsq_sim_free(rsq_sim *s) {
    if (s) {
        (void)hipSetDevice(s->device);
        if (s->mailbox) (void)hipHostFree(s->mailbox);
        for (hipStream_t st : s->side)
            if (st) (void)hipStreamDestroy(st);
        for (rsq_sim::Workspace &w : s->ws)
            if (w.text_done) (void)hipEventDestroy(w.text_done);
        for (hipEvent_t e : {s->ev_call, s->ev_fill, s->ev_emit})
            if (e) (void)hipEventDestroy(e);
    }
    delete s;
}

int rsq_sim_prepare(rsq_sim *s, uint64_t seed, uint64_t num_read_pairs, double coverage, int ref_bias_mode, const char *record_base_identifier, void *stream) {
    REQUIRE(s, "null simulator");
    return guard([&] {
        HIP_CHECK(hipSetDevice(s->device));
        DevicePrepass be(*s, stream);
        prepare(*s, s->up, be, seed, num_read_pairs, coverage, ref_bias_mode, record_base_identifier);
        return RSQ_OK;
    });
}

int rsq_sim_prepare_plan(rsq_sim *s, uint64_t seed, uint64_t num_read_pairs, double coverage, int ref_bias_mode, const char *record_base_identifier) {
    REQUIRE(s, "null argument");
    return guard([&] {
        HIP_CHECK(hipSetDevice(s->device));
        prepare_plan(*s, s->up, seed, num_read_pairs, coverage, ref_bias_mode, record_base_identifier);
        return RSQ_OK;
    });
}
int rsq_sim_bias_partials(rsq_sim *s, uint32_t block_lo, uint32_t block_hi, double *sums, double *maxes, size_t cap, size_t *n, void *stream) {
    REQUIRE(s && n, "null argument");
    REQUIRE(s->pre.planned, "rsq_sim_prepare_plan must run first");
    *n = (size_t)bias_chunks(s->pre.bias_plan);
    if (!sums && !maxes && !cap) return RSQ_OK;
    REQUIRE(sums && maxes && cap >= *n, "arrays too small");
    return guard([&] {
        HIP_CHECK(hipSetDevice(s->device));
        DevicePrepass be(*s, stream);
        prepare_bias_partials(*s, be, block_lo, block_hi, sums, maxes);
        return RSQ_OK;
    });
}
int rsq_sim_prepare_normalization(rsq_sim *s, const double *sums, const double *maxes, size_t n) {
    REQUIRE(s && sums && maxes, "null argument");
    return guard([&] {
        HIP_CHECK(hipSetDevice(s->device));
        prepare_normalization(*s, s->up, sums, maxes, n);
        return RSQ_OK;
    });
}
int rsq_sim_prepare_sys_errors(rsq_sim *s, uint32_t block_lo, uint32_t block_hi, const uint32_t in_state[2], uint32_t out_state[2], void *stream) {
    REQUIRE(s && in_state && out_state, "null argument");
    return guard([&] {
        HIP_CHECK(hipSetDevice(s->device));
        DevicePrepass be(*s, stream);
        prepare_sys_errors(*s, be, block_lo, block_hi, in_state, out_state);
        return RSQ_OK;
    });
}
int rsq_sim_prepare_finish(rsq_sim *s) {
    REQUIRE(s, "null argument");
    return guard([&] {
        HIP_CHECK(hipSetDevice(s->device));
        DevicePrepass be(*s, nullptr);
        prepare_finish(*s, be);
        return RSQ_OK;
    });
}

int rsq_sim_get_sequence_lengths(const rsq_sim *s, uint32_t *out, size_t cap, uint32_t *n_sequences) {
    REQUIRE(s && n_sequences && s->has_ref, "null argument, or a simulator without a reference");
    *n_sequences = (uint32_t)s->seq_len.size();
    if (out && cap >= s->seq_len.size()) memcpy(out, s->seq_len.data(), s->seq_len.size() * sizeof(uint32_t));
    else if (out) {
        g_last_error = "room for " + std::to_string(cap) + " lengths, the reference has " + std::to_string(s->seq_len.size()) + " sequences";
        return RSQ_ENOSPC;
    }
    return RSQ_OK;
}
__global__ void k_reference_sequence(DevSim S, uint32_t seq, uint32_t allele, uint32_t pos, VarStart from, uint32_t n, bool reversed, uint64_t *tmpl, uint32_t words, uint32_t *flag) {
    if (threadIdx.x || blockIdx.x) return;
    if (2u == S.variants_loaded) {
        const AlleleView a = allele_view(S, seq, allele);
        const int64_t h = from.start_variant_pos ? a.begin_of(a.entries_before(a.r.v[from.first_variant_id].pos)) + from.start_variant_pos : a.to_allele(pos);
        if (reversed ? h < (int64_t)n : h + (int64_t)n > a.length()) {
            *flag = 1u;
            return;
        }
        allele_template(a, pos, from, n, reversed, tmpl, words);
        return;
    }
    FragmentSrc src;
    src.words = hap_words(S, allele);
    src.word_off = S.seq_word_off[seq];
    src.first = pos;
    src.len = n;
    src.reverse = reversed;
    src.sys_ = nullptr;
    src.converted = nullptr;
    src.gc_prefix = nullptr;
    for (uint32_t w = 0; w < words; ++w) tmpl[w] = 0;
    for (uint32_t k = 0; k < n; ++k) tmpl[k >> 5] |= (uint64_t)src.ref(k) << ((k & 31u) * 2u);
}
int rsq_sim_reference_sequence(rsq_sim *s, uint32_t seq, uint32_t start_pos, uint32_t frag_length, int reversed, int32_t first_variant_id, uint32_t first_variant_pos, uint32_t allele,
                               uint8_t *out, size_t cap) {
    REQUIRE(s && out && s->has_ref && seq < s->dev.n_seqs, "null argument, a simulator without a reference, or no such sequence");
    REQUIRE(allele < (s->has_variants ? s->num_alleles : 1u), "no such allele");
    REQUIRE(frag_length <= (1u << 20) && cap >= frag_length, "room for fewer bases than asked for (at most 2^20 per call)");
    const uint32_t L = s->seq_len[seq];
    REQUIRE(reversed ? start_pos <= L : start_pos < L || 0 == frag_length, "start position outside the sequence");
    if (2 != s->variants_mode)
        REQUIRE(reversed ? frag_length <= start_pos : frag_length <= L - start_pos, "the stretch asked for leaves the sequence");
    if (first_variant_pos) {
        REQUIRE(2 == s->variants_mode, "a start inside inserted bases needs variants with insertions");
        const uint32_t n_var = s->var_ptr[seq + 1] - s->var_ptr[seq];
        REQUIRE(first_variant_id >= 0 && (uint32_t)first_variant_id < n_var && first_variant_pos <= s->variants[s->var_ptr[seq] + first_variant_id].len,
                "first_variant does not name bases of a variant of this sequence");
    }
    if (!frag_length) return RSQ_OK;
    return guard([&] {
        HIP_CHECK(hipSetDevice(s->device));
        const uint32_t words = (frag_length + 31u) / 32u;
        uint64_t *dev = nullptr;
        HIP_CHECK(hipMalloc(&dev, (size_t)(words + 1u) * sizeof(uint64_t)));
        std::vector<uint64_t> host(words + 1u, 0);
        hipError_t e = hipMemset(dev, 0, (size_t)(words + 1u) * sizeof(uint64_t));
        if (e == hipSuccess) {
            hipLaunchKernelGGL(k_reference_sequence, dim3(1), dim3(64), 0, nullptr, s->dev, seq, allele, start_pos, VarStart{first_variant_id, first_variant_pos}, frag_length, reversed != 0,
                               dev, words, reinterpret_cast<uint32_t *>(dev + words));
            e = hipGetLastError();
        }
        if (e == hipSuccess) e = hipMemcpy(host.data(), dev, host.size() * sizeof(uint64_t), hipMemcpyDeviceToHost);
        (void)hipFree(dev);
        HIP_CHECK(e);
        if (host[words]) {
            g_last_error = "the stretch asked for leaves the allele's sequence";
            return RSQ_EINVAL;
        }
        for (uint32_t k = 0; k < frag_length; ++k) out[k] = (uint8_t)((host[k >> 5] >> ((k & 31u) * 2u)) & 3u);
        return RSQ_OK;
    });
}
int rsq_sim_export_reference(rsq_sim *s, const char *path) {
    REQUIRE(s && path, "null argument");
    return guard([&] {
        HIP_CHECK(hipSetDevice(s->device));
        HIP_CHECK(hipDeviceSynchronize());
        export_reference(*s, s->up, path);
        return RSQ_OK;
    });
}
int rsq_sim_import_reference(rsq_sim *s, const char *path) {
    REQUIRE(s && path, "null argument");
    return guard([&] {
        HIP_CHECK(hipSetDevice(s->device));
        MappedFile m(path);
        import_reference(*s, s->up, m.data, m.size, path);
        return RSQ_OK;
    });
}
int rsq_sim_specialize(rsq_sim *s, int kind, int *specialized) {
    REQUIRE(s && specialized && (kind == 0 || kind == 1), "null argument, or a kind that is neither 0 (read pairs) nor 1 (seqToIllumina records)");
    return guard([&] {
        HIP_CHECK(hipSetDevice(s->device));
        const uint32_t mask = effective_fill_mask(s->dev.lds.mask, s->force_fill_mode);
        g_spec_note.clear();
        hipFunction_t fn = spec_kernel(*s, kind == 0 ? SpecKind::kReads : SpecKind::kRecords, mask, kind == 0 && s->has_variants, fill_is_binned(*s));
        if (kind == 1 && fn) fn = spec_kernel(*s, SpecKind::kRecords, mask, true, fill_is_binned(*s));
        *specialized = fn != nullptr;
        if (!s->specialize) g_spec_note = "option specialize is 0: the library's own instantiation of the read kernel runs";
        else if (!mask) g_spec_note = "the read kernel draws in double precision from device memory (no table image): nothing to compile for the profile";
        g_last_warning = g_spec_note;
        return RSQ_OK;
    });
}
int rsq_profile_compile_read_kernel(const rsq_profile *p, int kind, int with_variants, int binned, const char *arch, const char *out_path, size_t *code_bytes, double *seconds) {
    REQUIRE(p && arch && code_bytes && (kind == 0 || kind == 1), "null argument, or a kind that is neither 0 nor 1");
    struct HostArrays : Uploader {
        std::vector<std::unique_ptr<char[]>> owned;
        void *put_bytes(const void *data, size_t bytes) override {
            owned.emplace_back(new char[bytes + 8]);
            memcpy(owned.back().get(), data, bytes);
            return owned.back().get();
        }
        void *put_zeros(size_t bytes) override {
            owned.emplace_back(new char[bytes + 8]());
            return owned.back().get();
        }
        void write_bytes(void *dst, const void *src, size_t bytes) override { memcpy(dst, src, bytes); }
        void read_bytes(void *dst, const void *src, size_t bytes) override { memcpy(dst, src, bytes); }
    };
    int rc = guard([&] {
        HostArrays up;
        SimState s;
        s.prof = p->p;
        pack_tables(s, up);
        pack_profile(s, up);
        if (!s.dev.lds.mask) throw Error("the profile has no table image (" + s.plan_note + "): there is nothing to compile for it");
        const SpecVariant variant{kind == 0 ? SpecKind::kReads : SpecKind::kRecords, s.dev.lds.mask, kind == 0 && with_variants != 0, binned != 0 || s.dev.lds.binned != 0};
        const std::string path = out_path ? out_path : "";
        if (path.size() > 4 && path.compare(path.size() - 4, 4, ".hip") == 0) {
            const std::string program = spec_program(spec_literals(s.dev), variant);
            FILE *f = fopen(out_path, "wb");
            if (!f || fwrite(program.data(), 1, program.size(), f) != program.size()) throw Error(std::string("cannot write ") + out_path);
            fclose(f);
            *code_bytes = program.size();
            if (seconds) *seconds = 0.0;
            return RSQ_OK;
        }
        SpecCode c;
        std::string note;
        if (!spec_compile(s.dev, variant, arch, c, note)) throw Error(note);
        *code_bytes = c.code.size();
        if (seconds) *seconds = c.seconds;
        if (out_path && *out_path) {
            FILE *f = fopen(out_path, "wb");
            if (!f || fwrite(c.code.data(), 1, c.code.size(), f) != c.code.size()) throw Error(std::string("cannot write ") + out_path);
            fclose(f);
        }
        return RSQ_OK;
    });
    return rc;
}
int rsq_set_kernel_cache_dir(const char *path) {
    spec_cache_dir_override() = path ? path : "";
    spec_cache_dir_set() = true;
    return RSQ_OK;
}
int rsq_sim_get_fill_plan(const rsq_sim *s, uint32_t *quality_quads, uint32_t *image_tiles, uint32_t *image_bytes) {
    REQUIRE(s && quality_quads && image_tiles && image_bytes, "null argument");
    *quality_quads = effective_fill_mask(s->dev.lds.mask, s->force_fill_mode);
    *image_tiles = *quality_quads ? s->dev.lds.img_tiles : 0u;
    *image_bytes = *quality_quads ? s->dev.lds.total_words * 4u : 0u;
    return RSQ_OK;
}
int rsq_sim_get_info(const rsq_sim *s, rsq_sim_info *out) {
    REQUIRE(s && out && (s->prepared || s->pre.planned), "simulator not prepared");
    out->total_pairs = s->total_pairs;
    out->adapter_only_pairs = s->adapter_only_pairs;
// ... 683 lines not shown
    if (!any) return;
    s->cur->rec_count.reserve(16);
    uint32_t *flag = s->cur->rec_count.as<uint32_t>() + 2;
    uint32_t *mail = reinterpret_cast<uint32_t *>(&s->mailbox[6]);
    mail[0] = 0xFFFFFFFFu;
    HIP_CHECK(hipMemcpyAsync(flag, mail, 4, hipMemcpyHostToDevice, st));
    hipLaunchKernelGGL(k_fragment_range, dim3(cdiv(n, 256)), dim3(256), 0, st, seg_dev, frag_len_dev, n, range, flag);
    HIP_CHECK(hipGetLastError());
    HIP_CHECK(hipMemcpyAsync(mail, flag, 4, hipMemcpyDeviceToHost, st));
    HIP_CHECK(hipStreamSynchronize(st));
    const uint32_t bad = mail[0];
    if (bad == 0xFFFFFFFFu) return;
    uint32_t fl = 0;
    uint8_t seg = 0;
    HIP_CHECK(hipMemcpy(&fl, frag_len_dev + bad, 4, hipMemcpyDeviceToHost));
    HIP_CHECK(hipMemcpy(&seg, seg_dev + bad, 1, hipMemcpyDeviceToHost));
    const DevReadLengths &rl = s->dev.read_lengths[seg ? 1 : 0];
    const bool in_insert_lengths = fl >= s->insert_lengths_from && fl < s->dev.insert_to;
    const uint64_t from = in_insert_lengths ? rl.row_first : s->insert_lengths_from, to = in_insert_lengths ? (uint64_t)rl.row_first + rl.rows : s->dev.insert_to;
    throw FragmentLengthOutside("record " + std::to_string(bad) + " of the call: Called index " + std::to_string(fl) + " range is from " + std::to_string(from) + " to " + std::to_string(to) +
                                " (the fragment length has no entry in the profile's " + (in_insert_lengths ? "read lengths by fragment length" : "insert lengths") + ")");
}

static RawLayout error_model_fill(rsq_sim *s, uint64_t first_index, uint64_t n, uint32_t read_len, const uint8_t *seqs_dev, const uint8_t *seg_dev, const uint32_t *frag_len_dev,
                                  const uint8_t *dom_dev, const uint8_t *rate_dev, hipStream_t st, const uint32_t *rec_at = nullptr, const uint32_t *rec_len = nullptr,
                                  uint32_t array_bytes = 0, bool fresh_timers = true, const uint16_t *codes = nullptr) {
    const uint32_t need_ops = (s->rmax + read_len + s->max_adapter + 4u + 15u) / 16u;
    if (need_ops > s->ops_stride) s->ops_stride = need_ops;
    if (n >= 0xFFFFFFFFull) throw Error("at most 2^32-1 records per call");
    s->cur = &s->ws[0];
    if (fresh_timers) reset_call_timers(*s);
    check_fragment_lengths(s, n, seg_dev, frag_len_dev, st);
    RawLayout raw = raw_layout(*s, n);
    if (!fill_is_binned(*s)) {
        s->cur->rec_flags.reserve(n * 4 + 16);
        s->cur->rec_index.reserve(n * 4 + 16);
        s->cur->rec_count.reserve(8);
        s->cur->offsets.reserve((n + 1) * 8);
        const dim3 rgrid(cdiv(n, 256)), rblock(256);
        hipLaunchKernelGGL(k_record_flags, rgrid, rblock, 0, st, seg_dev, n, s->cur->rec_flags.as<uint32_t>());
        exclusive_scan(*s, s->cur->rec_flags.as<uint32_t>(), n, s->cur->offsets.as<uint64_t>(), st);
        hipLaunchKernelGGL(k_record_partition, rgrid, rblock, 0, st, seg_dev, n, s->cur->offsets.as<uint64_t>(), s->cur->rec_index.as<uint32_t>(), s->cur->rec_count.as<uint32_t>());
        HIP_CHECK(hipGetLastError());
    }
    const RecordJob job{first_index, read_len, seqs_dev, dom_dev, rate_dev, frag_len_dev, s->cur->rec_index.as<uint32_t>(), s->cur->rec_count.as<uint32_t>(), n, rec_at, rec_len, array_bytes, codes};
    raw.order = launch_fill_records(*s, job, seg_dev, n, raw, st);
    return raw;
}

int rsq_sim_error_model(rsq_sim *s, uint64_t first_index, uint64_t n, uint32_t read_len, const uint8_t *seqs_dev, const uint8_t *seg_dev, const uint32_t *frag_len_dev,
                        const uint8_t *dom_dev, const uint8_t *rate_dev, uint8_t *seq_out_dev, uint8_t *qual_out_dev, uint32_t out_stride, uint16_t *read_len_out_dev,
                        uint16_t *num_errors_out_dev, uint16_t *tile_out_dev, char *cigar_out_dev, uint32_t cigar_stride, void *stream) {
    REQUIRE(s && s->prepared, "simulator not prepared");
    REQUIRE(seqs_dev && seg_dev && frag_len_dev && dom_dev && rate_dev && seq_out_dev && qual_out_dev && read_len_out_dev && num_errors_out_dev && tile_out_dev && cigar_out_dev,
            "null device pointer");
    if (!n) return RSQ_OK;
    return guard([&] {
        hipStream_t st = (hipStream_t)stream;
        HIP_CHECK(hipSetDevice(s->device));
        const RawLayout raw = error_model_fill(s, first_index, n, read_len, seqs_dev, seg_dev, frag_len_dev, dom_dev, rate_dev, st);
        s->cur->scan_total.reserve(8);
        HIP_CHECK(hipMemsetAsync(s->cur->scan_total.as<uint32_t>(), 0, 4, st));
        if (!((out_stride | (uint32_t)(uintptr_t)seq_out_dev | (uint32_t)(uintptr_t)qual_out_dev) & 3u))
            hipLaunchKernelGGL(k_error_model_rows, dim3(cdiv(n * 16, 256)), dim3(256), 0, st, raw, n, seq_out_dev, qual_out_dev, out_stride);
        hipLaunchKernelGGL(k_error_model_out, dim3(cdiv(n, 64)), dim3(64), 0, st, raw, n, seq_out_dev, qual_out_dev, out_stride, read_len_out_dev, num_errors_out_dev,
                           tile_out_dev, cigar_out_dev, cigar_stride, s->cur->scan_total.as<uint32_t>());
        HIP_CHECK(hipGetLastError());
        uint32_t overflow = 0;
        HIP_CHECK(hipMemcpyAsync(&overflow, s->cur->scan_total.as<uint32_t>(), 4, hipMemcpyDeviceToHost, st));
        HIP_CHECK(hipStreamSynchronize(st));
        if (overflow) {
            g_last_error = "out_stride or cigar_stride too small for at least one record";
            return (int)RSQ_ENOSPC;
        }
        return (int)RSQ_OK;
    });
}

static int error_model_text(rsq_sim *s, const RawLayout &raw, uint64_t n, const RecordIds &ids, char *text_dev, size_t text_cap, size_t *text_len, hipStream_t st) {
    s->cur->sizes.reserve(n * 4 + 16);
    s->cur->off_r1.reserve((n + 1) * 8);
    s->timers["format_write"].start(st);
    hipLaunchKernelGGL(k_record_text_sizes, dim3(cdiv(n, 256)), dim3(256), 0, st, raw, n, ids, s->cur->sizes.as<uint32_t>());
    exclusive_scan(*s, s->cur->sizes.as<uint32_t>(), n, s->cur->off_r1.as<uint64_t>(), st);
    s->longest_record.reserve(8);
    HIP_CHECK(hipMemsetAsync(s->longest_record.as<uint32_t>(), 0, 4, st));
    hipLaunchKernelGGL(k_max_size, dim3(std::min<uint64_t>(1024, cdiv(n, 256))), dim3(256), 0, st, s->cur->sizes.as<uint32_t>(), n, s->longest_record.as<uint32_t>());
    const uint32_t lds = format_lds_bytes(s->record_text_bytes, raw.order != nullptr);
    launch_text_waves(k_record_text_waves<true>, k_record_text_waves<false>, raw.order, dim3(cdiv(n, kFormatRecords)), lds, st, raw, n, ids, s->cur->off_r1.as<uint64_t>(), text_dev,
                      (uint64_t)text_cap, lds);
    s->timers["format_write"].stop(st);
    HIP_CHECK(hipGetLastError());
    HIP_CHECK(hipMemcpyAsync(&s->mailbox[2], s->cur->off_r1.as<uint64_t>() + n, 8, hipMemcpyDeviceToHost, st));
    HIP_CHECK(hipMemcpyAsync(&s->mailbox[5], s->longest_record.as<uint32_t>(), 4, hipMemcpyDeviceToHost, st));
    HIP_CHECK(hipStreamSynchronize(st));
    *text_len = s->mailbox[2];
    if ((uint32_t)s->mailbox[5]) s->record_text_bytes = (uint32_t)s->mailbox[5] + 8u;
    if (*text_len > text_cap) {
        g_last_error = "text buffer too small: need " + std::to_string(*text_len) + " bytes";
        return (int)RSQ_ENOSPC;
    }
    return (int)RSQ_OK;
}

int rsq_sim_error_model_fastq(rsq_sim *s, uint64_t first_index, uint64_t n, uint32_t read_len, const uint8_t *seqs_dev, const uint8_t *seg_dev, const uint32_t *frag_len_dev,
                              const uint8_t *dom_dev, const uint8_t *rate_dev, const char *ids_dev, const uint64_t *id_off_dev, char *text_dev, size_t text_cap,
                              size_t *text_len, void *stream) {
    REQUIRE(s && s->prepared, "simulator not prepared");
    REQUIRE(seqs_dev && seg_dev && frag_len_dev && dom_dev && rate_dev && ids_dev && id_off_dev && text_len && (text_dev || !text_cap), "null pointer");
    *text_len = 0;
    if (!n) return RSQ_OK;
    return guard([&] {
        hipStream_t st = (hipStream_t)stream;
        HIP_CHECK(hipSetDevice(s->device));
        const RawLayout raw = error_model_fill(s, first_index, n, read_len, seqs_dev, seg_dev, frag_len_dev, dom_dev, rate_dev, st);
        return error_model_text(s, raw, n, RecordIds{ids_dev, id_off_dev, nullptr, nullptr}, text_dev, text_cap, text_len, st);
    });
}

static std::string record_message(const std::vector<uint8_t> &rec) {
    std::vector<uint8_t> scratch[3];
    for (auto &v : scratch) v.resize(rec.size() + 8);
    fasta::RecordFields f{0, 0, 0, 0};
    const fasta::RecordError e = fasta::parse_record(rec.data(), rec.size(), fasta::ByteArrays{scratch[0].data(), scratch[1].data(), scratch[2].data()}, f);
    const size_t line_end = (size_t)fasta::find_byte(rec.data(), 1, rec.size(), '\n');
    size_t header_len = line_end - 1;
    if (header_len && rec[line_end - 1] == '\r') --header_len;
    const std::string header(reinterpret_cast<const char *>(rec.data()) + 1, header_len);
    size_t L = 0;
    for (size_t p = line_end + 1; p < rec.size(); ++p)
        if (rec[p] != '\n' && !(rec[p] == '\r' && (p + 1 == rec.size() || rec[p + 1] == '\n'))) ++L;
    size_t end = header_len > 2 * L + 2 ? header_len - 2 * L - 3 : 0;
    while (end && header[end] != ' ') --end;
    switch (e) {
        case fasta::kTooShort: return "Read description is too short to contain systematic error information and a sequence id: " + header;
        case fasta::kErrorSeparators: return "The two systematic error entries are not separated by a semicolon from themselves or the rest of the ReSeq information: " + header;
        case fasta::kNoId: return "No sequence id found that is separated by a space from the ReSeq information: " + header;
        case fasta::kSegment: return std::string("Template segment is ") + header[end + 1] + " not 1 or 2: " + header;
        case fasta::kSegmentSeparator: return "The template segment and fragment length are not separated by a semicolon: " + header;
        case fasta::kFragmentLength: {
            const size_t fl_at = end + 3, fl_end = header_len - 2 * L - 2;
            return "Fragment length '" + (fl_end > fl_at ? header.substr(fl_at, fl_end - fl_at) : std::string()) + "' is not a pure integer: " + header;
        }
        case fasta::kContainsN: return "input sequences must not contain N: " + header.substr(0, end);
        default: return "malformed record: " + header;
    }
}

int rsq_sim_error_model_fasta(rsq_sim *s, uint64_t first_index, const char *text_dev, size_t text_len, int final, char *out_dev, size_t out_cap, size_t *out_len,
                              uint64_t *n_records, size_t *consumed, void *stream) {
    REQUIRE(s && s->prepared, "simulator not prepared");
    REQUIRE(out_len && n_records && consumed && (text_dev || !text_len) && (out_dev || !out_cap), "null pointer");
    REQUIRE(text_len < 0xFFFFFFF0ull, "a block of FASTA text has to be shorter than 4 GB");
    *out_len = 0;
    *n_records = 0;
    *consumed = 0;
    if (!text_len) return RSQ_OK;
    return guard([&] {
        hipStream_t st = (hipStream_t)stream;
        HIP_CHECK(hipSetDevice(s->device));
        s->cur = &s->ws[0];
        rsq_sim::Workspace &w = *s->cur;
        const uint8_t *text = reinterpret_cast<const uint8_t *>(text_dev);
        const uint32_t n_tiles = cdiv(text_len, fasta::kTileBytes);
        auto roomy = [](size_t bytes) { return bytes + bytes / 8 + 64; };
        w.fa_counts.reserve(roomy((size_t)n_tiles * 4));
        w.fa_first.reserve(roomy(((size_t)n_tiles + 1) * 8));
        w.fa_summary.reserve(64);
        const dim3 tgrid(cdiv(n_tiles, fasta::kStartsBlock / 64u)), tblock(fasta::kStartsBlock);
        hipLaunchKernelGGL(fasta::k_fasta_count, tgrid, tblock, 0, st, text, (uint64_t)text_len, n_tiles, w.fa_counts.as<uint32_t>());
// ... 357 lines not shown
```

Baseline: 236.1 million.

## Stage sieve gap tables in LDS, precompute bias tracks, fuse scan with max

Adds an LDS-staged variant of the sieve gap kernel that copies the per-length gap tables into shared memory when they fit, on by default through a new sieve_lds option. Adds optional precomputed start/end surrounding-bias tracks so the finish kernel can skip recomputing surrounding bias, and rewrites the exclusive scan to use wave shuffles, vectorized loads, 16 items per thread, and batching of two arrays. The scan also folds in the longest-record max reduction, which removes the separate k_max_size launches. Together these aim to cut global memory latency in the sieve and kernel-launch and reduction overhead in formatting, at the cost of added code paths and extra device memory for the tracks.

```diff
diff --git a/reseq_amd/csrc/rsq_core.h b/reseq_amd/csrc/rsq_core.h
--- a/reseq_amd/csrc/rsq_core.h
+++ b/reseq_amd/csrc/rsq_core.h
@@ -465,10 +465,9 @@
     }
     return count;
 }
-RSQ_HD uint32_t fragment_counts(const DevSim &S, uint32_t seq, uint32_t fragment_length, uint32_t gc, const uint32_t (&sur_start)[3],
-                                const uint32_t (&sur_end)[3], double probability_chosen) {
+RSQ_HD uint32_t fragment_counts_from(const DevSim &S, uint32_t seq, uint32_t fragment_length, uint32_t gc, double start_factor, double end_factor, double probability_chosen) {
     double general = S.ref_seq_bias[seq] * S.insert_lengths_bias[fragment_length];
-    double bias = general * S.gc_bias[gc] * surrounding_bias(S.sur_bias, sur_start) * surrounding_bias(S.sur_bias, sur_end);
+    double bias = general * S.gc_bias[gc] * start_factor * end_factor;
     if (0.0 < bias) {
         double mean = bias * S.bias_normalization;
         double dispersion = get_dispersion(mean, S.dispersion[0], S.dispersion[1]) / S.num_alleles;
@@ -476,6 +475,11 @@
         return negative_binomial(mean / (mean + dispersion), dispersion, probability_chosen);
     }
     return 0;
+}
+RSQ_HD uint32_t fragment_counts(const DevSim &S, uint32_t seq, uint32_t fragment_length, uint32_t gc, const uint32_t (&sur_start)[3],
+                                const uint32_t (&sur_end)[3], double probability_chosen) {
+    const double start_factor = surrounding_bias(S.sur_bias, sur_start), end_factor = surrounding_bias(S.sur_bias, sur_end);
+    return fragment_counts_from(S, seq, fragment_length, gc, start_factor, end_factor, probability_chosen);
 }
 
 
diff --git a/reseq_amd/csrc/rsq_format.h b/reseq_amd/csrc/rsq_format.h
--- a/reseq_amd/csrc/rsq_format.h
+++ b/reseq_amd/csrc/rsq_format.h
@@ -449,12 +449,6 @@
     const uint64_t want = (kFormatRecords * record_bytes + 16u + 127u) & ~(uint64_t)127u;
     const uint32_t image = (uint32_t)(want < kFormatLdsMin ? kFormatLdsMin : want > kFormatLdsMax ? kFormatLdsMax : want);
     return !slots ? image : image + 16u * kFormatRecords < kFormatLdsMax ? image + 16u * kFormatRecords : kFormatLdsMax;
-}
-__global__ void __launch_bounds__(256) k_max_size(const uint32_t *sizes, uint64_t n, uint32_t *longest) {
-    uint32_t m = 0;
-    for (uint64_t i = (uint64_t)blockIdx.x * blockDim.x + threadIdx.x; i < n; i += (uint64_t)gridDim.x * blockDim.x) m = max(m, sizes[i]);
-    for (uint32_t d = 32; d; d >>= 1) m = max(m, (uint32_t)__shfl_xor((int)m, (int)d, 64));
-    if ((threadIdx.x & 63u) == 0 && m) atomicMax(longest, m);
 }
 template <bool PERM>
 __global__ void __launch_bounds__(64) k_format_write(DevSim S, NameTable names, const Fragment *frags, uint64_t n_pairs, uint64_t adapter_only_first, RawLayout raw,
diff --git a/reseq_amd/csrc/rsq_host.cpp b/reseq_amd/csrc/rsq_host.cpp
--- a/reseq_amd/csrc/rsq_host.cpp
+++ b/reseq_amd/csrc/rsq_host.cpp
@@ -43,6 +43,7 @@
     {"serial_parse", &Options::serial_parse},   {"parse_stretch", &Options::parse_stretch}, {"mapped_parses", &Options::mapped_parses},
     {"fasta_stretch", &Options::fasta_stretch}, {"overlap", &Options::overlap}, {"specialize", &Options::specialize}, {"job_write_direct", &Options::job_write_direct},             {"job_chunk_bytes", &Options::job_chunk_bytes}, {"host_gzip", &Options::host_gzip}, {"fill_waves", &Options::fill_waves}, {"fasta_no_stage", &Options::fasta_no_stage},
     {"hiprtc_by_name", &Options::hiprtc_by_name}, {"gzip_route", &Options::gzip_route},       {"gzip_stretch", &Options::gzip_stretch},
+    {"sieve_lds", &Options::sieve_lds},         {"sieve_lds_bytes", &Options::sieve_lds_bytes}, {"sieve_tracks_mb", &Options::sieve_tracks_mb},
 };
 }
 bool set_option(const char *name, int64_t value) {
diff --git a/reseq_amd/csrc/rsq_host.h b/reseq_amd/csrc/rsq_host.h
--- a/reseq_amd/csrc/rsq_host.h
+++ b/reseq_amd/csrc/rsq_host.h
@@ -41,6 +41,9 @@
     int64_t gzip_route = -1;
     int64_t gzip_stretch = 0;
     int64_t hiprtc_by_name = 0;
+    int64_t sieve_lds = 1;
+    int64_t sieve_lds_bytes = 0;
+    int64_t sieve_tracks_mb = 4096;
     int64_t overlap = 0;
 };
 Options &options();
diff --git a/reseq_amd/csrc/rsq_scan.h b/reseq_amd/csrc/rsq_scan.h
--- a/reseq_amd/csrc/rsq_scan.h
+++ b/reseq_amd/csrc/rsq_scan.h
@@ -5,27 +5,80 @@
 
 #if RSQ_DEVICE_BUILD
 constexpr uint32_t kScanBlock = 256;
-constexpr uint32_t kScanPer = 8;
+constexpr uint32_t kScanPer = 16;
 constexpr uint32_t kScanTile = kScanBlock * kScanPer;
+constexpr uint32_t kScanRounds = kScanPer / 4u, kScanWaves = kScanBlock / 64u, kScanWaveSpan = 64u * kScanPer;
 
-__global__ void k_scan_tile_sums(const uint32_t *in, uint64_t n, uint64_t *tile_sums) {
-    __shared__ uint64_t s[kScanBlock];
-    uint64_t base = (uint64_t)blockIdx.x * kScanTile + (uint64_t)threadIdx.x * kScanPer, acc = 0;
-    for (uint32_t i = 0; i < kScanPer; ++i)
-        if (base + i < n) acc += in[base + i];
-    s[threadIdx.x] = acc;
+struct ScanArrays {
+    const uint32_t *in[2];
+    uint64_t *out[2];
+    const uint64_t *init[2];
+    uint64_t *total[2];
+};
+
+__device__ __forceinline__ uint4 scan_load4(const uint32_t *in, uint64_t at, uint64_t n, bool aligned) {
+    if (at + 4u <= n) {
+        if (aligned) return *reinterpret_cast<const uint4 *>(in + at);
+        return uint4{in[at], in[at + 1u], in[at + 2u], in[at + 3u]};
+    }
+    uint4 v{0u, 0u, 0u, 0u};
+    if (at < n) v.x = in[at];
+    if (at + 1u < n) v.y = in[at + 1u];
+    if (at + 2u < n) v.z = in[at + 2u];
+    return v;
+}
+__device__ __forceinline__ uint64_t scan_shfl_up(uint64_t v, uint32_t d) {
+    return (uint64_t)(uint32_t)__shfl_up((int)(uint32_t)v, d, 64) | ((uint64_t)(uint32_t)__shfl_up((int)(uint32_t)(v >> 32), d, 64) << 32);
+}
+__device__ __forceinline__ uint64_t scan_shfl(uint64_t v, int from) {
+    return (uint64_t)(uint32_t)__shfl((int)(uint32_t)v, from, 64) | ((uint64_t)(uint32_t)__shfl((int)(uint32_t)(v >> 32), from, 64) << 32);
+}
+__device__ __forceinline__ uint64_t scan_shfl_xor(uint64_t v, uint32_t d) {
+    return (uint64_t)(uint32_t)__shfl_xor((int)(uint32_t)v, (int)d, 64) | ((uint64_t)(uint32_t)__shfl_xor((int)(uint32_t)(v >> 32), (int)d, 64) << 32);
+}
+
+__global__ void __launch_bounds__(kScanBlock) k_scan_tile_sums(ScanArrays a, uint64_t n, uint64_t *tile_sums, uint32_t *longest) {
+    __shared__ uint64_t s_sum[kScanWaves];
+    __shared__ uint32_t s_max[kScanWaves];
+    const uint32_t *in = a.in[blockIdx.y];
+    const bool aligned = 0u == (reinterpret_cast<uintptr_t>(in) & 15u);
+    const uint32_t lane = threadIdx.x & 63u, wave = threadIdx.x >> 6;
+    const uint64_t base = (uint64_t)blockIdx.x * kScanTile + (uint64_t)wave * kScanWaveSpan + 4u * lane;
+    uint64_t acc = 0;
+    uint32_t m = 0;
+#pragma unroll
+    for (uint32_t k = 0; k < kScanRounds; ++k) {
+        const uint4 v = scan_load4(in, base + 256u * k, n, aligned);
+        acc += (uint64_t)v.x + v.y + v.z + v.w;
+        m = max(max(m, v.x), max(max(v.y, v.z), v.w));
+    }
+    for (uint32_t d = 32; d; d >>= 1) {
+        acc += scan_shfl_xor(acc, d);
+        m = max(m, (uint32_t)__shfl_xor((int)m, (int)d, 64));
+    }
+    if (0u == lane) {
+        s_sum[wave] = acc;
+        s_max[wave] = m;
+    }
     __syncthreads();
-    for (uint32_t d = kScanBlock / 2; d > 0; d >>= 1) {
-        if (threadIdx.x < d) s[threadIdx.x] += s[threadIdx.x + d];
-        __syncthreads();
+    if (0u == threadIdx.x) {
+        uint64_t sum = 0;
+        uint32_t mx = 0;
+        for (uint32_t w = 0; w < kScanWaves; ++w) {
+            sum += s_sum[w];
+            mx = max(mx, s_max[w]);
+        }
+        tile_sums[(uint64_t)blockIdx.y * gridDim.x + blockIdx.x] = sum;
+        if (longest && mx) atomicMax(longest, mx);
     }
-    if (threadIdx.x == 0) tile_sums[blockIdx.x] = s[0];
 }
 constexpr uint32_t kScanTilesBlock = 1024;
-__global__ void __launch_bounds__(kScanTilesBlock) k_scan_tiles(uint64_t *tile_sums, uint32_t n_tiles, uint64_t *total, const uint64_t *init) {
+__global__ void __launch_bounds__(kScanTilesBlock) k_scan_tiles(ScanArrays a, uint64_t *all_tile_sums, uint32_t n_tiles) {
     __shared__ uint64_t s[kScanTilesBlock];
+    uint64_t *tile_sums = all_tile_sums + (uint64_t)blockIdx.x * n_tiles;
+    const uint64_t *init = a.init[blockIdx.x];
     const uint64_t first = init ? *init : 0u;
-    const uint32_t per = (n_tiles + kScanTilesBlock - 1u) / kScanTilesBlock, lo = threadIdx.x * per, hi = lo + per < n_tiles ? lo + per : n_tiles;
+    const uint32_t per = (n_tiles + kScanTilesBlock - 1u) / kScanTilesBlock, lo = min(threadIdx.x * per, n_tiles), hi = lo + per < n_tiles ? lo + per : n_tiles;
     uint64_t acc = 0;
     for (uint32_t i = lo; i < hi; ++i) acc += tile_sums[i];
     s[threadIdx.x] = acc;
@@ -42,31 +95,54 @@
         tile_sums[i] = run;
         run += v;
     }
-    if (threadIdx.x == kScanTilesBlock - 1u) *total = first + s[threadIdx.x];
+    if (threadIdx.x == kScanTilesBlock - 1u) *a.total[blockIdx.x] = first + s[threadIdx.x];
 }
-__global__ void k_scan_apply(const uint32_t *in, uint64_t n, const uint64_t *tile_sums, const uint64_t *total, uint64_t *out) {
-    __shared__ uint64_t s[kScanBlock];
-    const uint64_t base = (uint64_t)blockIdx.x * kScanTile + (uint64_t)threadIdx.x * kScanPer;
-    uint32_t v[kScanPer];
-    uint64_t acc = 0;
-    for (uint32_t i = 0; i < kScanPer; ++i) {
-        v[i] = base + i < n ? in[base + i] : 0u;
-        acc += v[i];
+__global__ void __launch_bounds__(kScanBlock) k_scan_apply(ScanArrays a, uint64_t n, const uint64_t *tile_sums) {
+    __shared__ uint64_t s_wave[kScanWaves];
+    const uint32_t *in = a.in[blockIdx.y];
+    uint64_t *out = a.out[blockIdx.y];
+    const bool aligned = 0u == (reinterpret_cast<uintptr_t>(in) & 15u), out_aligned = 0u == (reinterpret_cast<uintptr_t>(out) & 15u);
+    const uint32_t lane = threadIdx.x & 63u, wave = threadIdx.x >> 6;
+    const uint64_t base = (uint64_t)blockIdx.x * kScanTile + (uint64_t)wave * kScanWaveSpan + 4u * lane;
+    uint4 v[kScanRounds];
+    uint64_t before[kScanRounds];
+    uint64_t run = 0;
+#pragma unroll
+    for (uint32_t k = 0; k < kScanRounds; ++k) v[k] = scan_load4(in, base + 256u * k, n, aligned);
+#pragma unroll
+    for (uint32_t k = 0; k < kScanRounds; ++k) {
+        const uint64_t mine = (uint64_t)v[k].x + v[k].y + v[k].z + v[k].w;
+        uint64_t incl = mine;
+        for (uint32_t d = 1; d < 64u; d <<= 1) {
+            const uint64_t t = scan_shfl_up(incl, d);
+            if (lane >= d) incl += t;
+        }
+        before[k] = run + incl - mine;
+        run += scan_shfl(incl, 63);
     }
-    s[threadIdx.x] = acc;
+    if (0u == lane) s_wave[wave] = run;
     __syncthreads();
-    for (uint32_t d = 1; d < kScanBlock; d <<= 1) {
-        uint64_t t = threadIdx.x >= d ? s[threadIdx.x - d] : 0;
-        __syncthreads();
-        s[threadIdx.x] += t;
-        __syncthreads();
+    uint64_t front = tile_sums[(uint64_t)blockIdx.y * gridDim.x + blockIdx.x];
+    for (uint32_t w = 0; w < wave; ++w) front += s_wave[w];
+#pragma unroll
+    for (uint32_t k = 0; k < kScanRounds; ++k) {
+        const uint64_t at = base + 256u * k;
+        uint64_t o = front + before[k];
+        if (at + 4u <= n && out_aligned) {
+            *reinterpret_cast<ulonglong2 *>(out + at) = ulonglong2{o, o + v[k].x};
+            o += (uint64_t)v[k].x + v[k].y;
+            *reinterpret_cast<ulonglong2 *>(out + at + 2u) = ulonglong2{o, o + v[k].z};
+        } else {
+            if (at < n) out[at] = o;
+            o += v[k].x;
+            if (at + 1u < n) out[at + 1u] = o;
+            o += v[k].y;
+            if (at + 2u < n) out[at + 2u] = o;
+            o += v[k].z;
+            if (at + 3u < n) out[at + 3u] = o;
+        }
     }
-    uint64_t run = tile_sums[blockIdx.x] + s[threadIdx.x] - acc;
-    for (uint32_t i = 0; i < kScanPer; ++i) {
-        if (base + i < n) out[base + i] = run;
-        run += v[i];
-    }
-    if (blockIdx.x == 0 && threadIdx.x == 0) out[n] = *total;
+    if (blockIdx.x == 0 && threadIdx.x == 0) out[n] = *a.total[blockIdx.y];
 }
 #endif
 
diff --git a/reseq_amd/csrc/rsq_sieve.h b/reseq_amd/csrc/rsq_sieve.h
--- a/reseq_amd/csrc/rsq_sieve.h
+++ b/reseq_amd/csrc/rsq_sieve.h
@@ -17,25 +17,34 @@
 
 RSQ_HD uint32_t site_c1(const SieveSite &site) { return site.seq | (site.sub << 22); }
 
-template <class F>
-RSQ_HD uint32_t sieve_gaps(const DevSim &S, const SieveSite &site, F &&on_pass) {
-    const double *q = S.gap_q + (size_t)site.group * S.insert_to;
-    const uint32_t *seg_end = S.gap_seg_end + (size_t)site.group * S.insert_to;
+struct GapTables {
+    const double *q_;
+    const uint32_t *seg_end_;
+    const double *thr_;
+    RSQ_HD double q(uint32_t len) const { return q_[len]; }
+    RSQ_HD uint32_t seg_end(uint32_t len) const { return seg_end_[len]; }
+    RSQ_HD double thr1(uint32_t len) const { return thr_[2u * len + 1u]; }
+};
+RSQ_HD GapTables gap_tables(const DevSim &S, const SieveSite &site) {
+    return GapTables{S.gap_q + (size_t)site.group * S.insert_to, S.gap_seg_end + (size_t)site.group * S.insert_to, site.thr};
+}
+template <class T, class F>
+RSQ_HD uint32_t sieve_gaps_in(const DevSim &S, const SieveSite &site, const T &tab, F &&on_pass) {
     const uint32_t c1 = site_c1(site);
     uint32_t cur = S.insert_from, k = 0, n = 0;
     while (cur < S.insert_to) {
         const Words w = philox(S.seed, site.start, c1, k++, kDomSieve << 28);
-        const uint32_t e = seg_end[cur];
-        const double base = (cur == S.insert_from || seg_end[cur - 1u] == cur) ? 1.0 : q[cur - 1u];
+        const uint32_t e = tab.seg_end(cur);
+        const double base = (cur == S.insert_from || tab.seg_end(cur - 1u) == cur) ? 1.0 : tab.q(cur - 1u);
         const double target = u53_to_unit(w.w0, w.w1) * base;
         uint32_t lo = cur, hi = e;
         while (lo < hi) {
             const uint32_t mid = (lo + hi) >> 1;
-            if (q[mid] <= target) hi = mid;
+            if (tab.q(mid) <= target) hi = mid;
             else lo = mid + 1u;
         }
         if (lo < e) {
-            const double thr1 = site.thr[2u * lo + 1u];
+            const double thr1 = tab.thr1(lo);
             on_pass(lo, thr1 + u53_to_unit(w.w2, w.w3) * (1 - thr1));
             ++n;
             cur = lo + 1u;
@@ -43,8 +52,23 @@
     }
     return n;
 }
-
-RSQ_HD uint32_t sieve_cell(const DevSim &S, SieveSite &site, uint32_t len, double probability_chosen, uint32_t (&cnt)[2], uint32_t (&strand_of)[2]) {
+template <class F>
+RSQ_HD uint32_t sieve_gaps(const DevSim &S, const SieveSite &site, F &&on_pass) {
+    return sieve_gaps_in(S, site, gap_tables(S, site), on_pass);
+}
+
+RSQ_HD void surrounding_factors(const DevSim &S, SieveSite &site, uint32_t end, double &start_factor, double &end_factor) {
+    if (!site.have_start) {
+        surrounding_forward(S.ref_words, site.word_off, site.L, site.start, site.sur_start);
+        site.have_start = true;
+    }
+    uint32_t sur_end[3];
+    surrounding_reverse(S.ref_words, site.word_off, site.L, end - 1u, sur_end);
+    start_factor = surrounding_bias(S.sur_bias, site.sur_start);
+    end_factor = surrounding_bias(S.sur_bias, sur_end);
+}
+template <class Factors>
+RSQ_HD uint32_t sieve_cell_with(const DevSim &S, SieveSite &site, uint32_t len, double probability_chosen, uint32_t (&cnt)[2], uint32_t (&strand_of)[2], Factors &&factors) {
     cnt[0] = cnt[1] = 0;
     strand_of[0] = strand_of[1] = 0;
     const double thr0 = site.thr[2u * len], thr1 = site.thr[2u * len + 1u];
@@ -62,21 +86,21 @@
         strand_of[1] = 1;
         n_chosen = 2;
     }
-    if (!site.have_start) {
-        surrounding_forward(S.ref_words, site.word_off, site.L, site.start, site.sur_start);
-        site.have_start = true;
-    }
-    uint32_t sur_end[3];
-    surrounding_reverse(S.ref_words, site.word_off, site.L, end - 1u, sur_end);
+    double start_factor, end_factor;
+    factors(site, end, start_factor, end_factor);
     const uint32_t gc = percent_u32(ref_gc_count_prefix(S.ref_words, S.gc_prefix, site.word_off, site.start, end), len);
     uint32_t n_here = 0;
     for (uint32_t j = 0; j < n_chosen; ++j) {
         const double u = j ? u53_to_unit(w2.w2, w2.w3) : u53_to_unit(w2.w0, w2.w1);
         const double adjusted_random = thr0 + u * (1 - thr0);
-        cnt[j] = fragment_counts(S, site.seq, len, gc, site.sur_start, sur_end, adjusted_random);
+        cnt[j] = fragment_counts_from(S, site.seq, len, gc, start_factor, end_factor, adjusted_random);
         n_here += cnt[j];
     }
     return n_here;
+}
+RSQ_HD uint32_t sieve_cell(const DevSim &S, SieveSite &site, uint32_t len, double probability_chosen, uint32_t (&cnt)[2], uint32_t (&strand_of)[2]) {
+    return sieve_cell_with(S, site, len, probability_chosen, cnt, strand_of,
+                           [&S](SieveSite &st, uint32_t end, double &start_factor, double &end_factor) { surrounding_factors(S, st, end, start_factor, end_factor); });
 }
 
 constexpr uint32_t kMaxDevAlleles = 128;
@@ -350,6 +374,18 @@
     }
 }
 
+template <bool FILL, class T>
+__device__ __forceinline__ void sieve_gaps_lane(const DevSim &S, const SieveSite &site, const T &tab, uint32_t slot, uint32_t *counts, const uint64_t *cand_off, SieveCand *cands,
+                                                uint64_t cand_cap) {
+    if constexpr (FILL) {
+        uint64_t at = cand_off[slot];
+        sieve_gaps_in(S, site, tab, [&](uint32_t len, double probability_chosen) {
+            if (at < cand_cap) cands[at] = SieveCand{slot, len, probability_chosen};
+            ++at;
+        });
+    } else counts[slot] = sieve_gaps_in(S, site, tab, [](uint32_t, double) {});
+}
+
 template <int VM, bool FILL>
 __global__ void __launch_bounds__(kSieveBlock) k_sieve_gaps(DevSim S, uint32_t block_lo, uint32_t block_hi, uint32_t n_slots, uint32_t *counts, const uint64_t *cand_off,
                                                             SieveCand *cands, uint64_t cand_cap, const SlotInfo *slots) {
@@ -361,19 +397,65 @@
         if constexpr (!FILL) counts[slot] = 0;
         return;
     }
-    if constexpr (FILL) {
-        uint64_t at = cand_off[slot];
-        sieve_gaps(S, site, [&](uint32_t len, double probability_chosen) {
-            if (at < cand_cap) cands[at] = SieveCand{slot, len, probability_chosen};
-            ++at;
-        });
-    } else counts[slot] = sieve_gaps(S, site, [](uint32_t, double) {});
-}
+    sieve_gaps_lane<FILL>(S, site, gap_tables(S, site), slot, counts, cand_off, cands, cand_cap);
+}
+
+constexpr uint32_t kSieveTilesPerGroup = 4;
+constexpr uint32_t kSieveLdsPerLength = 20;
+constexpr size_t kSieveLdsLimit = 64u << 10;
+struct GapTablesLds {
+    const double *q_, *thr1_;
+    const uint32_t *seg_end_;
+    uint32_t from;
+    __device__ double q(uint32_t len) const { return q_[len - from]; }
+    __device__ uint32_t seg_end(uint32_t len) const { return seg_end_[len - from]; }
+    __device__ double thr1(uint32_t len) const { return thr1_[len - from]; }
+};
+template <int VM, bool FILL>
+__global__ void __launch_bounds__(kSieveBlock) k_sieve_gaps_lds(DevSim S, uint32_t block_lo, uint32_t block_hi, uint32_t n_slots, uint32_t *counts, const uint64_t *cand_off,
+                                                                SieveCand *cands, uint64_t cand_cap, const SlotInfo *slots) {
+    extern __shared__ double s_gap_tables[];
+    const uint32_t from = S.insert_from, n_len = S.insert_to - from;
+    double *s_q = s_gap_tables, *s_thr1 = s_gap_tables + n_len;
+    uint32_t *s_seg_end = reinterpret_cast<uint32_t *>(s_gap_tables + 2u * n_len);
+    const GapTablesLds lds{s_q, s_thr1, s_seg_end, from};
+    const uint32_t n_tiles = (n_slots + kSieveBlock - 1u) / kSieveBlock;
+    const uint32_t tile_lo = blockIdx.x * kSieveTilesPerGroup, tile_hi = tile_lo + kSieveTilesPerGroup < n_tiles ? tile_lo + kSieveTilesPerGroup : n_tiles;
+    uint32_t staged = 0xFFFFFFFFu;
+    for (uint32_t tile = tile_lo; tile < tile_hi; ++tile) {
+        SieveSite first;
+        init_site_slot<VM, false>(S, block_lo, block_hi, tile * kSieveBlock, first, nullptr, slots);
+        if (first.group != staged) {
+            __syncthreads();
+            const GapTables mem = gap_tables(S, first);
+            for (uint32_t i = threadIdx.x; i < n_len; i += kSieveBlock) {
+                s_q[i] = mem.q(from + i);
+                s_thr1[i] = mem.thr1(from + i);
+                s_seg_end[i] = mem.seg_end(from + i);
+            }
+            staged = first.group;
+            __syncthreads();
+        }
+        const uint32_t slot = tile * kSieveBlock + threadIdx.x;
+        if (slot >= n_slots) continue;
+        SieveSite site;
+        init_site_slot<VM, false>(S, block_lo, block_hi, slot, site, nullptr, slots);
+        if (!(site.start < site.L)) {
+            if constexpr (!FILL) counts[slot] = 0;
+        } else if (site.group == staged) sieve_gaps_lane<FILL>(S, site, lds, slot, counts, cand_off, cands, cand_cap);
+        else sieve_gaps_lane<FILL>(S, site, gap_tables(S, site), slot, counts, cand_off, cands, cand_cap);
+    }
+}
+
+struct BiasTracks {
+    const double *start_bias, *end_bias;
+    uint64_t lo, hi;
+};
 
 template <int VM, uint32_t CAP = kMaxDevAlleles>
 __global__ void __launch_bounds__(kSieveBlock) k_sieve_finish(DevSim S, uint32_t block_lo, uint32_t block_hi, uint32_t n_slots, const uint64_t *cand_off, const SieveCand *cands,
                                                               uint64_t cand_cap, uint32_t *pairs_of, SieveHit *hits, uint32_t hit_cap, uint32_t *hit_count, const SlotInfo *slots,
-                                                              uint32_t *cell_info) {
+                                                              uint32_t *cell_info, BiasTracks tracks) {
     __shared__ uint32_t s_records, s_base;
     if (threadIdx.x == 0) s_records = 0;
     __syncthreads();
@@ -391,7 +473,13 @@
         else if constexpr (VM == 1) n_here = sieve_cell_var(S, site, cand.len, cand.probability_chosen, cell);
         else {
             uint32_t cnt[2], strand_of[2];
-            n_here = sieve_cell(S, site, cand.len, cand.probability_chosen, cnt, strand_of);
+            n_here = sieve_cell_with(S, site, cand.len, cand.probability_chosen, cnt, strand_of, [&](SieveSite &st, uint32_t end, double &start_factor, double &end_factor) {
+                const uint64_t at = S.seq_base_off[st.seq] + st.start, at_end = S.seq_base_off[st.seq] + end - 1u;
+                if (at >= tracks.lo && at_end < tracks.hi) {
+                    start_factor = tracks.start_bias[at - tracks.lo];
+                    end_factor = tracks.end_bias[at_end - tracks.lo];
+                } else surrounding_factors(S, st, end, start_factor, end_factor);
+            });
             cell.n = n_here ? 2u : 0u;
             for (uint32_t e = 0; e < 2u; ++e) {
                 cell.cnt[e] = (uint16_t)cnt[e];
diff --git a/reseq_amd/csrc/rsq_sim.hip b/reseq_amd/csrc/rsq_sim.hip
--- a/reseq_amd/csrc/rsq_sim.hip
+++ b/reseq_amd/csrc/rsq_sim.hip
@@ -11,6 +11,7 @@
 #include <chrono>
 #include <map>
 #include <thread>
+#include <type_traits>
 #include <memory>
 #include <string>
 #include <utility>
@@ -102,6 +103,7 @@
 struct Timer {
     std::vector<std::pair<hipEvent_t, hipEvent_t>> events;
     size_t used = 0;
+    size_t marks = 0;
     Timer() = default;
     Timer(const Timer &) = delete;
     Timer &operator=(const Timer &) = delete;
@@ -111,7 +113,8 @@
             (void)hipEventDestroy(e.second);
         }
     }
-    void reset() { used = 0; }
+    void reset() { used = marks = 0; }
+    void mark() { ++marks; }
     void start(hipStream_t st) {
         if (used == events.size()) {
             hipEvent_t a, b;
@@ -133,7 +136,7 @@
         }
         return sum;
     }
-    size_t launches() const { return used; }
+    size_t launches() const { return used + marks; }
 };
 
 }
@@ -270,6 +273,15 @@
     struct ChainBufs {
         DevBuf chains, chunk_chain, used, out[2], changed, list;
     } chain_bufs;
+    struct SieveTracks {
+        DevBuf start_bias, end_bias;
+        uint64_t lo = 0, hi = 0;
+        void drop() {
+            lo = hi = 0;
+            start_bias.release();
+            end_bias.release();
+        }
+    } sieve_tracks;
 };
 
 static bool fill_is_binned(const rsq_sim &s) { return effective_fill_mask(s.dev.lds.mask, s.force_fill_mode) != 0 && s.dev.lds.binned; }
@@ -303,7 +315,7 @@
         };
         const uint32_t n_chunks = bias_chunks(plan);
         if (!n_chunks) return;
-        DevBuf d_params, d_chunk_param, d_chunk_ptr, d_sum, d_max, d_start_bias, d_end_bias;
+        DevBuf d_params, d_chunk_param, d_chunk_ptr, d_sum, d_max, own_start_bias, own_end_bias;
         d_params.upload(plan.params);
         d_chunk_param.upload(plan.chunk_param);
         d_chunk_ptr.upload(plan.chunk_ptr);
@@ -316,6 +328,9 @@
         uint64_t window = kBiasWindow;
         if (s.opt.bias_window > 0) window = (uint64_t)s.opt.bias_window;
         const uint64_t reach = (uint64_t)kBiasBlock * kBiasRun + s.dev.insert_to, track_len = std::min(hi - lo, window) + reach;
+        s.sieve_tracks.drop();
+        const bool keep = 0 == s.variants_mode && hi - lo <= window && s.opt.sieve_tracks_mb > 0 && track_len * 16 <= ((uint64_t)s.opt.sieve_tracks_mb << 20);
+        DevBuf &d_start_bias = keep ? s.sieve_tracks.start_bias : own_start_bias, &d_end_bias = keep ? s.sieve_tracks.end_bias : own_end_bias;
         d_start_bias.reserve(track_len * 8 + 16);
         d_end_bias.reserve(track_len * 8 + 16);
         lap("track buffers");
@@ -326,6 +341,10 @@
             hipLaunchKernelGGL(k_sum_bias, dim3(n_chunks), dim3(kBiasBlock), 0, st, s.dev, d_params.as<BiasParam>(), d_chunk_param.as<uint32_t>(), d_chunk_ptr.as<uint32_t>(),
                                d_start_bias.as<double>(), d_end_bias.as<double>(), a, d_sum.as<double>(), d_max.as<double>(), a, b);
             HIP_CHECK(hipGetLastError());
+        }
+        if (keep) {
+            s.sieve_tracks.lo = lo;
+            s.sieve_tracks.hi = std::min<uint64_t>(s.total_ref_size, hi + reach);
         }
         lap("track and sum kernels");
         HIP_CHECK(hipMemcpyAsync(h_sum.data(), d_sum.as<double>(), h_sum.size() * 8, hipMemcpyDeviceToHost, st));
@@ -397,15 +416,20 @@
     }
 };
 
-static void exclusive_scan(rsq_sim &s, const uint32_t *in, uint64_t n, uint64_t *out, hipStream_t st, const uint64_t *init = nullptr, uint64_t *total_out = nullptr) {
+static void exclusive_scans(rsq_sim &s, ScanArrays a, uint32_t arrays, uint64_t n, hipStream_t st, uint32_t *longest = nullptr) {
     const uint32_t tiles = cdiv(n, kScanTile);
-    s.cur->tile_sums.reserve((size_t)(tiles + 1) * 8);
-    s.cur->scan_total.reserve(8);
-    uint64_t *total = total_out ? total_out : s.cur->scan_total.as<uint64_t>();
-    hipLaunchKernelGGL(k_scan_tile_sums, dim3(tiles), dim3(kScanBlock), 0, st, in, n, s.cur->tile_sums.as<uint64_t>());
-    hipLaunchKernelGGL(k_scan_tiles, dim3(1), dim3(kScanTilesBlock), 0, st, s.cur->tile_sums.as<uint64_t>(), tiles, total, init);
-    hipLaunchKernelGGL(k_scan_apply, dim3(tiles), dim3(kScanBlock), 0, st, in, n, s.cur->tile_sums.as<uint64_t>(), total, out);
+    s.cur->tile_sums.reserve((size_t)arrays * (tiles + 1) * 8);
+    s.cur->scan_total.reserve(16);
+    for (uint32_t i = 0; i < arrays; ++i)
+        if (!a.total[i]) a.total[i] = s.cur->scan_total.as<uint64_t>() + i;
+    uint64_t *tile_sums = s.cur->tile_sums.as<uint64_t>();
+    hipLaunchKernelGGL(k_scan_tile_sums, dim3(tiles, arrays), dim3(kScanBlock), 0, st, a, n, tile_sums, longest);
+    hipLaunchKernelGGL(k_scan_tiles, dim3(arrays), dim3(kScanTilesBlock), 0, st, a, tile_sums, tiles);
+    hipLaunchKernelGGL(k_scan_apply, dim3(tiles, arrays), dim3(kScanBlock), 0, st, a, n, (const uint64_t *)tile_sums);
     HIP_CHECK(hipGetLastError());
+}
+static void exclusive_scan(rsq_sim &s, const uint32_t *in, uint64_t n, uint64_t *out, hipStream_t st, const uint64_t *init = nullptr, uint64_t *total_out = nullptr, uint32_t *longest = nullptr) {
+    exclusive_scans(s, ScanArrays{{in, nullptr}, {out, nullptr}, {init, nullptr}, {total_out, nullptr}}, 1, n, st, longest);
 }
 
 static RawLayout raw_layout(rsq_sim &s, uint64_t n_reads) {
@@ -616,11 +640,11 @@
     w.off_r2.reserve((n_pairs + 1) * 8);
     uint64_t *totals = s.totals.as<uint64_t>();
     s.timers["scan"].start(st);
-    exclusive_scan(s, w.sizes.as<uint32_t>(), n_pairs, w.off_r1.as<uint64_t>(), st, totals + 2 * part, totals + 2 * (part + 1));
-    exclusive_scan(s, w.sizes.as<uint32_t>() + n_pairs, n_pairs, w.off_r2.as<uint64_t>(), st, totals + 2 * part + 1, totals + 2 * (part + 1) + 1);
+    exclusive_scans(s, ScanArrays{{w.sizes.as<uint32_t>(), w.sizes.as<uint32_t>() + n_pairs}, {w.off_r1.as<uint64_t>(), w.off_r2.as<uint64_t>()},
+                                  {totals + 2 * part, totals + 2 * part + 1}, {totals + 2 * (part + 1), totals + 2 * (part + 1) + 1}},
+                    2, n_pairs, st, s.longest_record.as<uint32_t>());
     s.timers["scan"].stop(st);
     const uint32_t lds = format_lds_bytes(s.format_record_bytes, rd.row_order != nullptr);
-    hipLaunchKernelGGL(k_max_size, dim3(std::min<uint64_t>(1024, cdiv(2 * n_pairs, 256))), dim3(256), 0, st, w.sizes.as<uint32_t>(), 2 * n_pairs, s.longest_record.as<uint32_t>());
     s.timers["format_write"].start(st);
     launch_text_waves(k_format_write<true>, k_format_write<false>, rd.row_order, dim3(cdiv(n_pairs, kFormatRecords), 2), lds, st, s.dev, s.names, frags, n_pairs, adapter_first, rd.raw,
                       w.off_r1.as<uint64_t>(), w.off_r2.as<uint64_t>(), r1, r2, (uint64_t)(r1 ? r1_cap : 0), (uint64_t)(r2 ? r2_cap : 0), fvars, rd.row_order, lds);
@@ -680,8 +704,7 @@
     hipLaunchKernelGGL(k_truth_sizes<Format>, dim3(cdiv(n_pairs, 256)), dim3(256), 0, st, s.dev, s.names, frags, n_pairs, adapter_first, rd.raw, rd.row_order, side.as<Pair>(),
                        w.sam_sizes.as<uint32_t>());
     s.timers[sizes_timer].stop(st);
-    exclusive_scan(s, w.sam_sizes.as<uint32_t>(), n_pairs, w.off_sam.as<uint64_t>(), st, totals + part, totals + part + 1);
-    hipLaunchKernelGGL(k_max_size, dim3(std::min<uint64_t>(1024, cdiv(n_pairs, 256))), dim3(256), 0, st, w.sam_sizes.as<uint32_t>(), n_pairs, s.sam_longest.as<uint32_t>());
+    exclusive_scan(s, w.sam_sizes.as<uint32_t>(), n_pairs, w.off_sam.as<uint64_t>(), st, totals + part, totals + part + 1, s.sam_longest.as<uint32_t>());
     const uint32_t lds = sam_lds_bytes(bam ? s.bam_pair_bytes : s.sam_pair_bytes, rd.row_order != nullptr);
     if (sam.sorted) dst = sorted_stage_room(s, n_pairs, part, st, cap);
     s.timers[write_timer].start(st);
@@ -787,36 +810,50 @@
     const uint32_t block_lo = r.block_lo, block_hi = r.block_hi;
     const uint64_t n_slots = r.n_slots, cand_cap = r.cand_cap;
     const dim3 ggrid(cdiv(n_slots, kSieveBlock)), gblock(kSieveBlock);
+    const size_t lds_bytes = (size_t)(s.dev.insert_to - s.dev.insert_from) * kSieveLdsPerLength;
+    const bool in_lds = s.opt.sieve_lds != 0 && lds_bytes <= (s.opt.sieve_lds_bytes > 0 ? (size_t)s.opt.sieve_lds_bytes : kSieveLdsLimit);
+    const dim3 lgrid(cdiv(ggrid.x, kSieveTilesPerGroup));
+    const SlotInfo *slot_table = r.slot_table;
+    auto gaps = [&](auto vm_tag, auto fill_tag, uint32_t *counts, const uint64_t *cand_off, SieveCand *cands) {
+        constexpr int kVm = decltype(vm_tag)::value;
+        constexpr bool kFill = decltype(fill_tag)::value;
+        if (in_lds)
+            hipLaunchKernelGGL((k_sieve_gaps_lds<kVm, kFill>), lgrid, gblock, lds_bytes, st, s.dev, block_lo, block_hi, (uint32_t)n_slots, counts, cand_off, cands, cand_cap, slot_table);
+        else
+            hipLaunchKernelGGL((k_sieve_gaps<kVm, kFill>), ggrid, gblock, 0, st, s.dev, block_lo, block_hi, (uint32_t)n_slots, counts, cand_off, cands, cand_cap, slot_table);
+    };
+    using Vm0 = std::integral_constant<int, 0>;
+    using Vm2 = std::integral_constant<int, 2>;
     if (!attempt) {
         if (2 == vm) {
             w.slot_table.reserve(n_slots * sizeof(SlotInfo) + 16);
             s.timers["slot_table"].start(st);
             hipLaunchKernelGGL(k_slot_table, dim3(block_hi - block_lo), dim3(256), 0, st, s.dev, block_lo, w.slot_table.as<SlotInfo>());
             s.timers["slot_table"].stop(st);
-            r.slot_table = w.slot_table.as<SlotInfo>();
+            slot_table = r.slot_table = w.slot_table.as<SlotInfo>();
         }
         s.timers["sieve_screen"].start(st);
-        if (2 == vm)
-            hipLaunchKernelGGL((k_sieve_gaps<2, false>), ggrid, gblock, 0, st, s.dev, block_lo, block_hi, (uint32_t)n_slots, w.counts.as<uint32_t>(), (const uint64_t *)nullptr,
-                               (SieveCand *)nullptr, cand_cap, r.slot_table);
-        else
-            hipLaunchKernelGGL((k_sieve_gaps<0, false>), ggrid, gblock, 0, st, s.dev, block_lo, block_hi, (uint32_t)n_slots, w.counts.as<uint32_t>(), (const uint64_t *)nullptr,
-                               (SieveCand *)nullptr, cand_cap, r.slot_table);
+        if (2 == vm) gaps(Vm2{}, std::false_type{}, w.counts.as<uint32_t>(), nullptr, nullptr);
+        else gaps(Vm0{}, std::false_type{}, w.counts.as<uint32_t>(), nullptr, nullptr);
         s.timers["sieve_screen"].stop(st);
         exclusive_scan(s, w.counts.as<uint32_t>(), n_slots, w.offsets.as<uint64_t>(), st);
     }
-    const SlotInfo *slot_table = r.slot_table;
-    if (2 == vm)
-        hipLaunchKernelGGL((k_sieve_gaps<2, true>), ggrid, gblock, 0, st, s.dev, block_lo, block_hi, (uint32_t)n_slots, (uint32_t *)nullptr, w.offsets.as<uint64_t>(),
-                           w.cands.as<SieveCand>(), cand_cap, slot_table);
-    else
-        hipLaunchKernelGGL((k_sieve_gaps<0, true>), ggrid, gblock, 0, st, s.dev, block_lo, block_hi, (uint32_t)n_slots, (uint32_t *)nullptr, w.offsets.as<uint64_t>(),
-                           w.cands.as<SieveCand>(), cand_cap, slot_table);
+    s.timers[in_lds ? "sieve_gaps_lds" : "sieve_gaps_mem"].mark();
+    if (2 == vm) gaps(Vm2{}, std::true_type{}, nullptr, w.offsets.as<uint64_t>(), w.cands.as<SieveCand>());
+    else gaps(Vm0{}, std::true_type{}, nullptr, w.offsets.as<uint64_t>(), w.cands.as<SieveCand>());
     const dim3 fgrid(cdiv(cand_cap, kSieveBlock)), fblock(kSieveBlock);
+    BiasTracks tracks{nullptr, nullptr, 0, 0};
+    if (0 == vm && s.sieve_tracks.hi > s.sieve_tracks.lo) {
+        auto global_of_block = [&](uint32_t b) { return s.seq_base_off[s.block_seq[b]] + (uint64_t)(b - s.first_block[s.block_seq[b]]) * kBlockSize; };
+        const uint64_t first = global_of_block(block_lo), last = std::min<uint64_t>(s.total_ref_size, global_of_block(block_hi - 1u) + kBlockSize + s.dev.insert_to);
+        if (first >= s.sieve_tracks.lo && last <= s.sieve_tracks.hi)
+            tracks = BiasTracks{s.sieve_tracks.start_bias.as<double>(), s.sieve_tracks.end_bias.as<double>(), s.sieve_tracks.lo, s.sieve_tracks.hi};
+    }
+    if (0 == vm) s.timers[tracks.hi > tracks.lo ? "sieve_tracks" : "sieve_tracks_off"].mark();
 #define RSQ_FINISH(VM, CAP)                                                                                                                                   \
     hipLaunchKernelGGL((k_sieve_finish<VM, CAP>), fgrid, fblock, 0, st, s.dev, block_lo, block_hi, (uint32_t)n_slots, w.offsets.as<uint64_t>(), w.cands.as<SieveCand>(),  \
                        cand_cap, w.pairs_of.as<uint32_t>(), w.hits.as<SieveHit>(), (uint32_t)std::min<uint64_t>(r.hit_cap, 0xFFFFFFFFull), w.hit_count.as<uint32_t>(), slot_table, \
-                       w.cell_info.as<uint32_t>())
+                       w.cell_info.as<uint32_t>(), tracks)
     if (2 == vm && s.num_alleles <= 8) RSQ_FINISH(2, 8);
     else if (2 == vm) RSQ_FINISH(2, kMaxDevAlleles);
     else if (1 == vm) RSQ_FINISH(1, 8);
@@ -1534,6 +1571,7 @@
     return guard([&] {
         HIP_CHECK(hipSetDevice(s->device));
         DevicePrepass be(*s, stream);
+        s->sieve_tracks.drop();
         prepare(*s, s->up, be, seed, num_read_pairs, coverage, ref_bias_mode, record_base_identifier);
         return RSQ_OK;
     });
@@ -1543,6 +1581,7 @@
     REQUIRE(s, "null argument");
     return guard([&] {
         HIP_CHECK(hipSetDevice(s->device));
+        s->sieve_tracks.drop();
         prepare_plan(*s, s->up, seed, num_read_pairs, coverage, ref_bias_mode, record_base_identifier);
         return RSQ_OK;
     });
@@ -1674,6 +1713,7 @@
     return guard([&] {
         HIP_CHECK(hipSetDevice(s->device));
         MappedFile m(path);
+        s->sieve_tracks.drop();
         import_reference(*s, s->up, m.data, m.size, path);
         return RSQ_OK;
     });
@@ -2523,10 +2563,9 @@
     s->cur->off_r1.reserve((n + 1) * 8);
     s->timers["format_write"].start(st);
     hipLaunchKernelGGL(k_record_text_sizes, dim3(cdiv(n, 256)), dim3(256), 0, st, raw, n, ids, s->cur->sizes.as<uint32_t>());
-    exclusive_scan(*s, s->cur->sizes.as<uint32_t>(), n, s->cur->off_r1.as<uint64_t>(), st);
     s->longest_record.reserve(8);
     HIP_CHECK(hipMemsetAsync(s->longest_record.as<uint32_t>(), 0, 4, st));
-    hipLaunchKernelGGL(k_max_size, dim3(std::min<uint64_t>(1024, cdiv(n, 256))), dim3(256), 0, st, s->cur->sizes.as<uint32_t>(), n, s->longest_record.as<uint32_t>());
+    exclusive_scan(*s, s->cur->sizes.as<uint32_t>(), n, s->cur->off_r1.as<uint64_t>(), st, nullptr, nullptr, s->longest_record.as<uint32_t>());
     const uint32_t lds = format_lds_bytes(s->record_text_bytes, raw.order != nullptr);
     launch_text_waves(k_record_text_waves<true>, k_record_text_waves<false>, raw.order, dim3(cdiv(n, kFormatRecords)), lds, st, raw, n, ids, s->cur->off_r1.as<uint64_t>(), text_dev,
                       (uint64_t)text_cap, lds);
```

Measured after the change: 244.8 million, median of 6. 3.7% higher.
